# VideoVerses/VideoTuna-dev

Measured on AMD Instinct MI355X. Metric: finetune samples/sec, CogVideoX-2B T2V LoRA 49x480x720 bf16, higher is better.
Workload: dtype bf16; 1 GPU; CogVideoX-2B T2V LoRA finetune 49x480x720 (configs[1]): latents [4,13,16,60,90], text [4,226,4096], r=4 LoRA on to_q/k/v/out, 4 samples per optimizer step as in the YAML (batch_size 2 x accumulate_grad_batches 2), run as 1 micro-batch(es) of 4; mode=lora, model=CogVideoX-2B, micro_batch=4, accumulate_grad_batches=1, global_batch=4, seq_len=17776, layers=30, parallelism=dp1, recompute=none (107 GB of block activations kept in HBM), weights=seeded random init (no checkpoints offline), text=pre-encoded prompt embeddings (synthetic), latents=pre-encoded latents (synthetic)

## Files before the change

include/vt355.h:

```cpp
#ifndef VT355_H
#define VT355_H
#ifdef __cplusplus
extern "C" {
#endif

#define VT_OK 0
#define VT_ERR_BAD_SHAPE (-1)
#define VT_ERR_BAD_ALIGN (-2)
#define VT_ERR_LAUNCH (-3)
#define VT_ERR_UNSUPPORTED (-4)

int vt_version(void);
const char* vt_arch(void);
const char* vt_error_string(int code);

#define VT_EPI_BIAS 0
#define VT_EPI_BIAS_GELU 1
#define VT_EPI_GATED_RES 2
#define VT_EPI_DGELU 3

int vt_gemm_bf16(const void* A, int lda, const void* W, int ldw, void* C, int ldc,
                 int M, int N, int K, const void* bias, int epilogue, int out_fp32,
                 const void* R, int ldr, int r_mod,
                 const float* gate_txt, const float* gate_vid, int gate_bstride, int S, int St,
                 void* C2, int ldc2, const void* U, int ldu, void* stream);
int vt_gemm_set_tile(int mode);
int vt_gemm_bf16_kernel(int M, int N, int K);
int vt_conv_set_tile(int mode);

int vt_gemm_nt_bf16(const void* A, int lda, const void* B, int ldb, float* C, int ldc, int M, int P, int Q,
                    float alpha, int accumulate, void* stream);
int vt_gemm_nt_bf16_unpad(const void* A, int lda, const void* B, int ldb, float* C, int ldc, int M, int P, int Q,
                          float alpha, int accumulate, int row_group, int row_keep, int col_group, int col_keep, void* stream);

int vt_group_colsum(const void* X, int ldx, const void* Y, int ldy, const float* mean, const float* rstd,
                    float* out1, float* out2, long long M, int D, int S, int St, int grouped,
                    long long o_bstride, long long o_segstride, void* stream);

int vt_qk_ln_param_grads(const float* dq_hat, int lddq, const void* dk_hat, int lddk, const void* qkv, int ld,
                         const float* mean, const float* rstd, float* out_2x2x64, long long M, int H,
                         const float* rope_cos, const float* rope_sin, int S, int St, void* stream);
int vt_ln_param_combine(const float* G1, const float* G2, int G, int D, const void* gamma, const void* beta,
                        const float* scale_txt, const float* scale_vid, int bstride, float* dgamma, float* dbeta,
                        float* dshift_txt, float* dshift_vid, float* dscale_txt, float* dscale_vid, int dbstride,
                        int grouped, void* stream);
int vt_small_linear_bwd(const float* dy, int ldy, const void* x, int ldx, const void* W, float* dW, float* db,
                        float* dx, int lddx, int Bn, int N, int K, void* stream);
int vt_silu_bwd(const float* dy, const void* x, float* dx, long long n, void* stream);

int vt_attn_fwd_hd64(const void* q, const void* k, const void* v, void* o, float* lse2,
                     int B, int H, int S,
                     long long q_rs, long long k_rs, long long v_rs, long long o_rs,
                     long long q_bs, long long k_bs, long long v_bs, long long o_bs,
                     float softmax_scale, int q_prescaled, void* stream);

int vt_attn_fwd_bias_hd64(const void* q, const void* k, const void* v, const float* bias_t, void* o, float* lse2,
                          int B, int H, int S,
                          long long q_rs, long long k_rs, long long v_rs, long long o_rs,
                          long long q_bs, long long k_bs, long long v_bs, long long o_bs,
                          float softmax_scale, void* stream);
int vt_gemm_splitk_f32(const void* A, int lda, const void* W, int ldw, float* C, int ldc, int M, int N, int K, int splits, void* stream);
int vt_residual_cast_bf16(const float* acc, long long lda, const void* R, long long ldr, void* out, long long ldo, long long M, int N,
                          void* stream);
long long vt_groupnorm_ws_bytes(int N, int C);
int vt_groupnorm_silu_cl(const void* x, long long ldx, const void* gamma, const void* beta, void* y, long long ldy,
                         int N, long long P, int C, int G, float eps, int silu, float* ws, long long ws_bytes, void* stream);
int vt_causal_conv3d_cl(const void* x, long long ldx, const void* wk, const void* bias, const void* res, long long ldr,
                        void* y, long long ldy, int N, int T, int H, int W, int Cin, int Cout, void* stream);
int vt_downsample_conv2d_cl(const void* x, long long ldx, const void* wk, const void* bias, void* y, long long ldy,
                            int N, int T, int H, int W, int Cin, int Cout, void* stream);
int vt_causal_conv3d_in8_cl(const void* x, const void* wk, const void* bias, void* y, long long ldy,
                            int N, int T, int H, int W, int Cout, void* stream);
int vt_temporal_pool_cl(const void* x, long long ldx, void* y, long long ldy, int N, int T, long long HW, int C, int keep_first,
                        void* stream);
int vt_rmsnorm_bf16(const void* x, long long ldx, const void* w, void* y, long long ldy, long long M, int D, float eps,
                    void* stream);
int vt_gated_gelu_bf16(const void* u, long long ldu, void* y, long long ldy, long long M, int F, void* stream);

int vt_attn_bwd_hd64(const void* q, const void* k, const void* v, const void* o, const void* dout,
                     const float* lse2, float* delta_ws, float* dq_f32, void* dk, void* dv,
                     int B, int H, int S,
                     long long q_rs, long long k_rs, long long v_rs, long long o_rs, long long do_rs,
                     long long dq_rs, long long dk_rs, long long dv_rs,
                     long long q_bs, long long k_bs, long long v_bs, long long o_bs, long long do_bs,
                     long long dq_bs, long long dk_bs, long long dv_bs,
                     float softmax_scale, int q_prescaled, void* chain_ws, long long chain_ws_bytes, void* stream);
long long vt_attn_bwd_chain_ws_bytes(int B, int H, int S);
int vt_attn_bwd_set_chain(int chain_len, int slots);

int vt_ln_modulate_fwd(const void* x, int ldx, void* y, int ldy, const void* gamma, const void* beta,
                       const float* shift_txt, const float* scale_txt, const float* shift_vid,
                       const float* scale_vid, int mod_bstride, float* mean, float* rstd,
                       int M, int D, int S, int St, float eps, void* stream);
int vt_ln_modulate_bwd(const void* dy, int lddy, const void* x, int ldx, const float* mean, const float* rstd,
                       const void* gamma, const float* scale_txt, const float* scale_vid, int mod_bstride,
                       const void* dres, int lddres, void* dx, int lddx,
                       int M, int D, int S, int St, void* stream);

int vt_qk_layernorm_fwd(const void* qkv, int ld, void* out, int ldo, const void* gq, const void* bq,
                        const void* gk, const void* bk, float* mean, float* rstd,
                        long long M, int H, float eps, float q_scale,
                        const float* rope_cos, const float* rope_sin, int S, int St, void* stream);
int vt_qk_layernorm_bwd(const float* dq_hat, int lddq, const void* dk_hat, int lddk, const void* qkv, int ld,
                        const float* mean, const float* rstd, const void* gq, const void* gk,
                        void* dqkv, int ldd, long long M, int H,
                        const float* rope_cos, const float* rope_sin, int S, int St, void* stream);

int vt_gate_mul(const void* x, int ldx, void* y, int ldy, const float* g_txt, const float* g_vid, int bstride,
                long long M, int D, int S, int St, void* stream);
int vt_silu_bf16(const void* x, void* y, long long n, void* stream);
int vt_cast_f32_bf16(const float* x, void* y, long long n, void* stream);
int vt_timestep_embedding(const long long* t, void* out, int B, int D, int flip_sin_to_cos, float freq_shift,
                          void* stream);
int vt_patchify(const void* img, void* tok, int B, int F, int C, int H, int W, int P, int ldt, void* stream);
int vt_unpatchify(const void* tok, void* img, int B, int F, int C, int H, int W, int P, int ldt, void* stream);

int vt_add_noise(const float* x0, const float* noise, const float* sqrt_ab, const float* sqrt_1mab, void* noisy,
                 long long per_sample, int B, void* stream);
int vt_diffusion_loss(const void* vpred, const void* noisy, const float* x0, const float* sqrt_ab,
                      const float* sqrt_1mab, const float* weights, float* loss, float* partials_ws,
                      void* dvpred, long long per_sample, int B, float grad_scale, void* stream);

int vt_diffusion_loss_bwd(const void* vpred, const void* noisy, const float* x0, const float* sqrt_ab,
                          const float* sqrt_1mab, const float* weights, const float* grad_out, void* dvpred,
                          long long per_sample, int B, void* stream);

int vt_adamw(float* p, const float* g, float* m, float* v, void* p_bf16, long long n, float lr, float beta1,
             float beta2, float eps, float weight_decay, int step, float grad_scale, const int* guard, void* stream);

int vt_grad_sqnorm_partials(void);
int vt_grad_sqnorm(const float* g, long long n, float* partials, int slot, void* stream);
int vt_clip_finalize(const float* partials, int nslots, float grad_scale, float max_norm, float* record, void* stream);
int vt_adamw_clip(float* p, const float* g, float* m, float* v, void* p_bf16, long long n, float lr, float beta1,
                  float beta2, float eps, float weight_decay, int step, float grad_scale, const int* guard,
                  const float* clip_coef_dev, float clip_value, void* stream);

int vt_lora_down(const void* X, int ldx, const void* A, int lda, int R, void* T, int ldt, long long M, int K,
                 int zero_cols, void* stream);
int vt_skinny_tn(const void* Big, int ldb, const void* Small, int lds_, int R, float* out, long long osp,
                 long long osr, float alpha, long long M, int P, float* workspace, void* stream);
long long vt_skinny_tn_workspace_bytes(int P);
int vt_lora_up_add(void* dX, int ldx, const void* dT, int ldt, const void* A, int lda, int R, long long M, int K,
                   void* stream);
int vt_lora_pack_b(const float* Bcat, void* Wext, int ldw, int n_adapters, int d_out, int r, float scale, void* stream);
int vt_lora_pack_bt(const float* Bcat, void* WText, int ldwt, int n_adapters, int d_out, int r, float scale, void* stream);

int vt_lora_down_wide(const void* X, int ldx, const void* A, int lda, int n_adapters, int r, int rp, int ext, void* T, int ldt,
                      long long M, int K, void* stream);
int vt_lora_tn_wide(const void* Big, int ldb, const void* Small, int lds_, int R, float* out, long long osp, long long osr,
                    float alpha, long long M, int P, void* stream);
int vt_lora_up_add_wide(void* dX, int ldx, const void* dT, int ldt, const void* A, int lda, int n_adapters, int r, int rp,
                        long long M, int K, void* stream);
int vt_lora_pack_b_wide(const float* Bcat, void* Wext, int ldw, int n_adapters, int d_out, int r, int rp, int ext, float scale,
                        void* stream);
int vt_lora_pack_bt_wide(const float* Bcat, void* WText, int ldwt, int n_adapters, int d_out, int r, int rp, int ext, float scale,
                         void* stream);

int vt_lora_down_drop(const void* X, int ldx, const void* A, int lda, int R, int n_adapters, void* T, int ldt, long long M, int K,
                      int zero_cols, float p, unsigned long long seed, int site0, void* stream);
int vt_skinny_tn_drop(const void* Big, int ldb, const void* Small, int lds_, int R, int n_adapters, float* out, long long osp,
                      long long osr, float alpha, long long M, int P, float* workspace, float p, unsigned long long seed, int site0,
                      void* stream);
int vt_lora_up_add_drop(void* dX, int ldx, const void* dT, int ldt, const void* A, int lda, int R, int n_adapters, long long M, int K,
                        float p, unsigned long long seed, int site0, void* stream);
int vt_lora_down_wide_drop_fits(int n_adapters, int rp);
int vt_lora_down_wide_drop(const void* X, int ldx, const void* A, int lda, int n_adapters, int r, int rp, int ext, void* T, int ldt,
                           long long M, int K, float p, unsigned long long seed, int site0, void* stream);
int vt_lora_tn_wide_drop(const void* Big, int ldb, const void* Small, int lds_, int R, float* out, long long osp, long long osr,
                         float alpha, long long M, int P, float p, unsigned long long seed, int site, void* stream);
int vt_lora_up_add_wide_drop(void* dX, int ldx, const void* dT, int ldt, const void* A, int lda, int n_adapters, int r, int rp,
                             long long M, int K, float p, unsigned long long seed, int site0, void* stream);
int vt_lora_up_add_dgelu_drop(void* dX, int ldx, const void* dT, int ldt, const void* A, int lda, int R, int n_adapters, const void* U,
                              int ldu, long long M, int K, float p, unsigned long long seed, int site0, void* stream);
int vt_lora_up_add_wide_dgelu_drop(void* dX, int ldx, const void* dT, int ldt, const void* A, int lda, int n_adapters, int r, int rp,
                                   const void* U, int ldu, long long M, int K, float p, unsigned long long seed, int site0, void* stream);

int vt_dora_norm(const void* W, int ldw, const void* A, int lda, const void* B, int n_adapters, int d_out, int r, int K, float scale,
                 const float* mag, float* out, void* stream);
int vt_dora_scale(const void* src, long long lds_, void* dst, long long ldd, const float* c, int rows, int cols, int by_col, void* stream);
int vt_dora_transpose_scale(const void* src, long long src_ld, void* dst, long long dst_ld, const float* c, int rows, int cols,
                            void* stream);
int vt_dora_db_add(float* G, const float* S, const float* c, int N, int r, void* stream);
int vt_dora_dm(const float* sum_g, const float* sum_gy, const void* bias, const float* mag, float* dm, int N, void* stream);


int vt_conv_cl(const void* x, long long ldx, const void* wk, const void* bias, const float* sbias, int sbias_ld,
               const void* res, long long ldr, void* y, long long ldy,
               int N, int T, int H, int W, int Cin, int Cout, int KT, int KH, int KW, int pt, int ph, int pw, int stride, void* stream);
int vt_conv_dw_cl(const void* dy, long long lddy, const void* x, long long ldx, float* dw,
                  int N, int T, int H, int W, int Cin, int Cout, int KT, int KH, int KW, int pt, int ph, int pw, int stride,
                  int accumulate, void* stream);
int vt_conv_dw_bias_cl(const void* dy, long long lddy, const void* x, long long ldx, float* dw, float* dbias,
                       int N, int T, int H, int W, int Cin, int Cout, int KT, int KH, int KW, int pt, int ph, int pw, int stride,
                       int accumulate, void* stream);
int vt_transpose_bf16(const void* src, long long src_ld, long long src_boff, void* dst, long long dst_ld, long long dst_boff, int rows, int cols,
                      int nb, void* stream);
int vt_transpose_multi_bf16(const void* table, int njobs, long long total_blocks, void* stream);
int vt_conv_desc_extents(long long ldx, long long lddy, int N, int T, int H, int W, int Cin, int Cout, int KH, int KW, int ph, int pw,
                         int stride, long long* fwd_x_bytes, long long* dw_x_bytes, long long* dw_dy_bytes);
int vt_groupnorm_silu_bwd_cl(const void* dy, long long lddy, const void* x, long long ldx, const void* gamma,
                             const float* ws_fwd, float* ws_bwd, long long ws_bytes, void* dx, long long lddx,
                             float* dgamma, float* dbeta, int N, long long P, int C, int G, int silu, int accumulate, void* stream);
int vt_geglu_fwd(const void* h, long long ldh, void* y, long long ldy, long long M, int F, void* stream);
int vt_geglu_bwd(const void* dy, long long lddy, const void* h, long long ldh, void* dh, long long lddh, long long M, int F, void* stream);
int vt_add_rows_bf16(const void* a, long long lda, const void* b, long long ldb, void* out, long long ldo, long long M, int C, void* stream);
int vt_dropout_bf16(const void* x, long long ldx, void* y, long long ldy, long long M, int C, float p, unsigned long long seed,
                    unsigned long long offset, void* mask_out, void* stream);
int vt_row_map_bf16(const void* src, long long lds, void* out, long long ldo, int mode, long long nb, int d1, int d2, int C,
                    int accumulate, void* stream);
int vt_q_sample(const float* x0, const float* noise, const float* sqrt_ab, const float* sqrt_1mab, const float* scale, void* xt,
                long long per_sample, int B, void* stream);
int vt_mse_loss(const void* pred, const float* target, float* loss, void* dpred, long long total, float grad_scale, void* stream);

int vt_attn_small_fwd(const void* q, const void* k, const void* v, void* o, float* lse2, int NB, int H, int Sq, int Sk,
                      long long q_rs, long long q_bs, long long k_rs, long long k_bs, long long v_rs, long long v_bs,
                      long long o_rs, long long o_bs, float softmax_scale, int mask_block, void* stream);
int vt_attn_small_bwd(const void* q, const void* k, const void* v, const void* o, const void* dout, const float* lse2,
                      void* dq, void* dk, void* dv, float* dk32, float* dv32, int NB, int H, int Sq, int Sk,
                      long long q_rs, long long q_bs, long long k_rs, long long k_bs, long long v_rs, long long v_bs,
                      long long o_rs, long long o_bs, long long do_rs, long long do_bs, long long dq_rs, long long dq_bs,
                      long long dk_rs, long long dv_rs, float softmax_scale, int mask_block, void* stream);

long long vt_attn_dual_ws_floats(int B, int H, int Sq, int rows_per_frame, int Sa, int Sb);
int vt_attn_dual_fwd(const void* q, const void* k, const void* v, const void* k_ip, const void* v_ip, void* o, float* lse2,
                     int B, int H, int Sq, int rows_per_frame, int Sa, int Sb,
                     long long q_rs, long long q_bs, long long k_rs, long long k_bs, long long v_rs, long long v_bs,
                     long long kip_rs, long long kip_bs, long long vip_rs, long long vip_bs, long long o_rs, long long o_bs,
                     float softmax_scale, float img_scale, void* stream);
int vt_attn_dual_bwd(const void* q, const void* k, const void* v, const void* k_ip, const void* v_ip, const void* dout,
                     const float* lse2, void* dq, float* dk32, float* dv32, float* dkip32, float* dvip32, float* ws,
                     long long ws_floats, int B, int H, int Sq, int rows_per_frame, int Sa, int Sb,
                     long long q_rs, long long q_bs, long long k_rs, long long k_bs, long long v_rs, long long v_bs,
                     long long kip_rs, long long kip_bs, long long vip_rs, long long vip_bs, long long do_rs, long long do_bs,
                     long long dq_rs, long long dq_bs, float softmax_scale, float img_scale, void* stream);

int vt_attn_gen_fwd(const void* q, const void* k, const void* v, void* o, float* lse2, const int* kv_len, int head_dim, int hstride,
                    int NB, int H, int Sq, int Sk, long long q_rs, long long q_bs, long long k_rs, long long k_bs, long long v_rs,
                    long long v_bs, long long o_rs, long long o_bs, float softmax_scale, int mask_block, void* stream);
int vt_attn_gen_bwd(const void* q, const void* k, const void* v, const void* o, const void* dout, const float* lse2, const int* kv_len,
                    void* dq, void* dk, void* dv, float* dk32, float* dv32, int head_dim, int hstride, int NB, int H, int Sq, int Sk,
                    long long q_rs, long long q_bs, long long k_rs, long long k_bs, long long v_rs, long long v_bs,
                    long long o_rs, long long o_bs, long long do_rs, long long do_bs, long long dq_rs, long long dq_bs,
                    long long dk_rs, long long dv_rs, float softmax_scale, int mask_block, void* stream);

int vt_opensora_loss(const float* out, const float* x0, const float* noise, const double* coef, double* loss3, float* dout,
                     long long per_channel, int C, int B, float grad_scale, void* stream);

int vt_gemm_fp8(const void* A, int lda, const void* W, int ldw, void* C, int ldc, int M, int N, int K, const void* bias,
                const float* scale_a, const float* scale_w, void* stream);
int vt_quantize_fp8(const void* x, long long ldx, void* y, long long ldy, long long M, int K, float* scale, unsigned int* ws,
                    int given_scale, void* stream);

int vt_gemm_mxfp8(const void* A, int lda, const void* W, int ldw, void* C, int ldc, int M, int N, int K, const void* bias,
                  const float* scale_a, const float* scale_w, int epilogue, const void* residual, int ldr,
                  const float* gate_txt, const float* gate_vid, int gate_bstride, int S, int St, void* pre_act_out, int ldc2,
                  const void* At, int ldat, const void* Wt, int ldwt, int Kt, void* Cq, int ldcq, const float* scale_out,
                  unsigned int* amax, void* stream);
int vt_cast_fp8_scaled(const void* x, long long ldx, void* y, long long ldy, void* cp, long long ldcp, long long M, int K, int L,
                       int Lj, int off, const float* scale, unsigned int* amax, void* stream);
int vt_ln_modulate_fwd_fp8(const void* x, int ldx, void* y, int ldy, const void* gamma, const void* beta,
                           const float* shift_txt, const float* scale_txt, const float* shift_vid,
                           const float* scale_vid, int mod_bstride, float* mean, float* rstd,
                           int M, int D, int S, int St, float eps, void* q, int ldq, const float* qscale, unsigned int* amax,
                           void* stream);
int vt_fp8_scale_update(unsigned int* amax, float* history, float* scale, int n, int H, void* stream);
int vt_gemm_mxfp8_dx(const void* G, int ldg, int fmt_g, const void* WT, int ldw, void* C, int ldc, int M, int N, int K,
                     const float* scale_g, const float* scale_w, int epilogue, const void* residual, int ldr,
                     const void* pre_act_in, int ldu, const void* At, int ldat, const void* Wt, int ldwt, int Kt,
                     void* Cq, int ldcq, int fmt_out, const float* scale_out, unsigned int* amax, void* stream);
int vt_cast_fp8_fmt(const void* x, long long ldx, void* y, long long ldy, void* cp, long long ldcp, long long M, int K, int L,
                    int Lj, int off, int fmt, const float* scale, unsigned int* amax, void* stream);
int vt_gate_mul_fp8(const void* x, int ldx, void* y, int ldy, const float* g_txt, const float* g_vid, int bstride, long long M,
                    int D, int S, int St, void* q, int ldq, int fmt, const float* scale, unsigned int* amax, void* stream);
int vt_fp8_scale_update_fmax(unsigned int* amax, float* history, float* scale, int n, int H, float fmax, void* stream);

int vt_qk_rmsnorm_rope128_fwd(const void* qkv, long long ld, void* out, long long ldo, const void* gq, const void* gk, float* rstd,
                              const float* rope_cos, const float* rope_sin, long long M, int H, int L, int Lout, int row_off,
                              int S_rope, float eps, void* stream);
int vt_qk_rmsnorm_rope128_bwd(const void* dout, long long lddo, const void* qkv, long long ld, void* dqkv, long long ldd, const void* gq,
                              const void* gk, const float* rstd, const float* rope_cos, const float* rope_sin, float* dgq, float* dgk,
                              long long M, int H, int L, int Lout, int row_off, int S_rope, void* stream);

int vt_attn128_fwd(const void* q, const void* k, const void* v, void* o, float* lse2, const int* kv_len, int B, int H, int S,
                   long long q_rs, long long k_rs, long long v_rs, long long o_rs,
                   long long q_bs, long long k_bs, long long v_bs, long long o_bs, float softmax_scale, void* stream);
int vt_attn128_bwd(const void* q, const void* k, const void* v, const void* o, const void* dout, const float* lse2, const int* kv_len,
                   float* delta_ws, float* dq32, void* dq_bf16, void* dk, void* dv, int B, int H, int S,
                   long long q_rs, long long k_rs, long long v_rs, long long o_rs, long long do_rs, long long dq_rs, long long dqb_rs,
                   long long dk_rs, long long dv_rs, long long q_bs, long long k_bs, long long v_bs, long long o_bs, long long do_bs,
                   long long dq_bs, long long dqb_bs, long long dk_bs, long long dv_bs, float softmax_scale, void* stream);

#ifdef __cplusplus
}
#endif
#endif
```

videotuna-dev_amd/_lib.py:

```python
import ctypes as C
import os

_HERE = os.path.dirname(os.path.abspath(__file__))
_LIB = None


class VtError(RuntimeError):
    pass


def lib_path() -> str:
    return os.environ.get("VT355_LIB") or os.path.join(_HERE, "libvt355.so")


_vp, _i, _ll, _f, _fp = C.c_void_p, C.c_int, C.c_longlong, C.c_float, C.c_void_p
PROTOTYPES = {
    "vt_version": [],
    "vt_arch": [],
    "vt_error_string": [_i],
    "vt_gemm_bf16": [_vp, _i, _vp, _i, _vp, _i, _i, _i, _i, _vp, _i, _i, _vp, _i, _i, _fp, _fp, _i, _i, _i,
                     _vp, _i, _vp, _i, _vp],
    "vt_gemm_set_tile": [_i],
    "vt_gemm_bf16_kernel": [_i, _i, _i],
    "vt_conv_set_tile": [_i],
    "vt_transpose_bf16": [_vp, _ll, _ll, _vp, _ll, _ll, _i, _i, _i, _vp],
    "vt_transpose_multi_bf16": [_vp, _i, _ll, _vp],
    "vt_gemm_nt_bf16": [_vp, _i, _vp, _i, _fp, _i, _i, _i, _i, _f, _i, _vp],
    "vt_gemm_nt_bf16_unpad": [_vp, _i, _vp, _i, _fp, _i, _i, _i, _i, _f, _i, _i, _i, _i, _i, _vp],
    "vt_group_colsum": [_vp, _i, _vp, _i, _fp, _fp, _fp, _fp, _ll, _i, _i, _i, _i, _ll, _ll, _vp],
    "vt_qk_ln_param_grads": [_fp, _i, _vp, _i, _vp, _i, _fp, _fp, _fp, _ll, _i, _fp, _fp, _i, _i, _vp],
    "vt_ln_param_combine": [_fp, _fp, _i, _i, _vp, _vp, _fp, _fp, _i, _fp, _fp, _fp, _fp, _fp, _fp, _i, _i, _vp],
    "vt_small_linear_bwd": [_fp, _i, _vp, _i, _vp, _fp, _fp, _fp, _i, _i, _i, _i, _vp],
    "vt_silu_bwd": [_fp, _vp, _fp, _ll, _vp],
    "vt_attn_fwd_hd64": [_vp, _vp, _vp, _vp, _fp, _i, _i, _i, _ll, _ll, _ll, _ll, _ll, _ll, _ll, _ll, _f, _i, _vp],
    "vt_attn_fwd_bias_hd64": [_vp, _vp, _vp, _fp, _vp, _fp, _i, _i, _i, _ll, _ll, _ll, _ll, _ll, _ll, _ll, _ll, _f, _vp],
    "vt_gemm_splitk_f32": [_vp, _i, _vp, _i, _fp, _i, _i, _i, _i, _i, _vp],
    "vt_residual_cast_bf16": [_fp, _ll, _vp, _ll, _vp, _ll, _ll, _i, _vp],
    "vt_groupnorm_ws_bytes": [_i, _i],
    "vt_groupnorm_silu_cl": [_vp, _ll, _vp, _vp, _vp, _ll, _i, _ll, _i, _i, _f, _i, _fp, _ll, _vp],
    "vt_causal_conv3d_cl": [_vp, _ll, _vp, _vp, _vp, _ll, _vp, _ll, _i, _i, _i, _i, _i, _i, _vp],
    "vt_causal_conv3d_in8_cl": [_vp, _vp, _vp, _vp, _ll, _i, _i, _i, _i, _i, _vp],
    "vt_downsample_conv2d_cl": [_vp, _ll, _vp, _vp, _vp, _ll, _i, _i, _i, _i, _i, _i, _vp],
    "vt_temporal_pool_cl": [_vp, _ll, _vp, _ll, _i, _i, _ll, _i, _i, _vp],
    "vt_rmsnorm_bf16": [_vp, _ll, _vp, _vp, _ll, _ll, _i, _f, _vp],
    "vt_gated_gelu_bf16": [_vp, _ll, _vp, _ll, _ll, _i, _vp],
    "vt_attn_bwd_hd64": [_vp, _vp, _vp, _vp, _vp, _fp, _fp, _fp, _vp, _vp, _i, _i, _i,
                         _ll, _ll, _ll, _ll, _ll, _ll, _ll, _ll, _ll, _ll, _ll, _ll, _ll, _ll, _ll, _ll, _f, _i, _vp, _ll, _vp],
    "vt_attn_bwd_chain_ws_bytes": [_i, _i, _i],
    "vt_attn_bwd_set_chain": [_i, _i],
    "vt_ln_modulate_fwd": [_vp, _i, _vp, _i, _vp, _vp, _fp, _fp, _fp, _fp, _i, _fp, _fp, _i, _i, _i, _i, _f, _vp],
    "vt_ln_modulate_bwd": [_vp, _i, _vp, _i, _fp, _fp, _vp, _fp, _fp, _i, _vp, _i, _vp, _i, _i, _i, _i, _i, _vp],
    "vt_qk_layernorm_fwd": [_vp, _i, _vp, _i, _vp, _vp, _vp, _vp, _fp, _fp, _ll, _i, _f, _f, _fp, _fp, _i, _i, _vp],
    "vt_qk_layernorm_bwd": [_fp, _i, _vp, _i, _vp, _i, _fp, _fp, _vp, _vp, _vp, _i, _ll, _i, _fp, _fp, _i, _i, _vp],
    "vt_gate_mul": [_vp, _i, _vp, _i, _fp, _fp, _i, _ll, _i, _i, _i, _vp],
    "vt_silu_bf16": [_vp, _vp, _ll, _vp],
    "vt_cast_f32_bf16": [_fp, _vp, _ll, _vp],
    "vt_timestep_embedding": [_vp, _vp, _i, _i, _i, _f, _vp],
    "vt_patchify": [_vp, _vp, _i, _i, _i, _i, _i, _i, _i, _vp],
    "vt_unpatchify": [_vp, _vp, _i, _i, _i, _i, _i, _i, _i, _vp],
    "vt_add_noise": [_fp, _fp, _fp, _fp, _vp, _ll, _i, _vp],
    "vt_diffusion_loss": [_vp, _vp, _fp, _fp, _fp, _fp, _fp, _fp, _vp, _ll, _i, _f, _vp],
    "vt_diffusion_loss_bwd": [_vp, _vp, _fp, _fp, _fp, _fp, _fp, _vp, _ll, _i, _vp],
    "vt_adamw": [_fp, _fp, _fp, _fp, _vp, _ll, _f, _f, _f, _f, _f, _i, _f, _vp, _vp],
    "vt_grad_sqnorm_partials": [],
    "vt_grad_sqnorm": [_fp, _ll, _fp, _i, _vp],
    "vt_clip_finalize": [_fp, _i, _f, _f, _fp, _vp],
    "vt_adamw_clip": [_fp, _fp, _fp, _fp, _vp, _ll, _f, _f, _f, _f, _f, _i, _f, _vp, _fp, _f, _vp],
    "vt_lora_down": [_vp, _i, _vp, _i, _i, _vp, _i, _ll, _i, _i, _vp],
    "vt_skinny_tn": [_vp, _i, _vp, _i, _i, _fp, _ll, _ll, _f, _ll, _i, _fp, _vp],
    "vt_skinny_tn_workspace_bytes": [_i],
    "vt_lora_up_add": [_vp, _i, _vp, _i, _vp, _i, _i, _ll, _i, _vp],
    "vt_lora_pack_b": [_fp, _vp, _i, _i, _i, _i, _f, _vp],
    "vt_lora_pack_bt": [_fp, _vp, _i, _i, _i, _i, _f, _vp],
    "vt_lora_down_wide": [_vp, _i, _vp, _i, _i, _i, _i, _i, _vp, _i, _ll, _i, _vp],
    "vt_lora_tn_wide": [_vp, _i, _vp, _i, _i, _fp, _ll, _ll, _f, _ll, _i, _vp],
    "vt_lora_up_add_wide": [_vp, _i, _vp, _i, _vp, _i, _i, _i, _i, _ll, _i, _vp],
    "vt_lora_pack_b_wide": [_fp, _vp, _i, _i, _i, _i, _i, _i, _f, _vp],
    "vt_lora_pack_bt_wide": [_fp, _vp, _i, _i, _i, _i, _i, _i, _f, _vp],
    "vt_lora_down_drop": [_vp, _i, _vp, _i, _i, _i, _vp, _i, _ll, _i, _i, _f, C.c_ulonglong, _i, _vp],
    "vt_skinny_tn_drop": [_vp, _i, _vp, _i, _i, _i, _fp, _ll, _ll, _f, _ll, _i, _fp, _f, C.c_ulonglong, _i, _vp],
    "vt_lora_up_add_drop": [_vp, _i, _vp, _i, _vp, _i, _i, _i, _ll, _i, _f, C.c_ulonglong, _i, _vp],
    "vt_lora_down_wide_drop_fits": [_i, _i],
    "vt_lora_down_wide_drop": [_vp, _i, _vp, _i, _i, _i, _i, _i, _vp, _i, _ll, _i, _f, C.c_ulonglong, _i, _vp],
    "vt_lora_tn_wide_drop": [_vp, _i, _vp, _i, _i, _fp, _ll, _ll, _f, _ll, _i, _f, C.c_ulonglong, _i, _vp],
    "vt_lora_up_add_wide_drop": [_vp, _i, _vp, _i, _vp, _i, _i, _i, _i, _ll, _i, _f, C.c_ulonglong, _i, _vp],
    "vt_lora_up_add_dgelu_drop": [_vp, _i, _vp, _i, _vp, _i, _i, _i, _vp, _i, _ll, _i, _f, C.c_ulonglong, _i, _vp],
    "vt_lora_up_add_wide_dgelu_drop": [_vp, _i, _vp, _i, _vp, _i, _i, _i, _i, _vp, _i, _ll, _i, _f, C.c_ulonglong, _i, _vp],
    "vt_dora_norm": [_vp, _i, _vp, _i, _vp, _i, _i, _i, _i, _f, _fp, _fp, _vp],
    "vt_dora_scale": [_vp, _ll, _vp, _ll, _fp, _i, _i, _i, _vp],
    "vt_dora_transpose_scale": [_vp, _ll, _vp, _ll, _fp, _i, _i, _vp],
    "vt_dora_db_add": [_fp, _fp, _fp, _i, _i, _vp],
    "vt_dora_dm": [_fp, _fp, _vp, _fp, _fp, _i, _vp],
    "vt_conv_cl": [_vp, _ll, _vp, _vp, _fp, _i, _vp, _ll, _vp, _ll] + [_i] * 13 + [_vp],
    "vt_conv_dw_cl": [_vp, _ll, _vp, _ll, _fp] + [_i] * 13 + [_i, _vp],
    "vt_conv_dw_bias_cl": [_vp, _ll, _vp, _ll, _fp, _fp] + [_i] * 13 + [_i, _vp],
    "vt_conv_desc_extents": [_ll, _ll] + [_i] * 11 + [C.POINTER(C.c_longlong)] * 3,
    "vt_groupnorm_silu_bwd_cl": [_vp, _ll, _vp, _ll, _vp, _fp, _fp, _ll, _vp, _ll, _fp, _fp, _i, _ll, _i, _i, _i, _i, _vp],
    "vt_geglu_fwd": [_vp, _ll, _vp, _ll, _ll, _i, _vp],
    "vt_geglu_bwd": [_vp, _ll, _vp, _ll, _vp, _ll, _ll, _i, _vp],
    "vt_add_rows_bf16": [_vp, _ll, _vp, _ll, _vp, _ll, _ll, _i, _vp],
    "vt_dropout_bf16": [_vp, _ll, _vp, _ll, _ll, _i, _f, C.c_ulonglong, C.c_ulonglong, _vp, _vp],
    "vt_row_map_bf16": [_vp, _ll, _vp, _ll, _i, _ll, _i, _i, _i, _i, _vp],
    "vt_q_sample": [_fp, _fp, _fp, _fp, _fp, _vp, _ll, _i, _vp],
    "vt_mse_loss": [_vp, _fp, _fp, _vp, _ll, _f, _vp],
    "vt_attn_small_fwd": [_vp, _vp, _vp, _vp, _fp, _i, _i, _i, _i] + [_ll] * 8 + [_f, _i, _vp],
    "vt_qk_rmsnorm_rope128_fwd": [_vp, _ll, _vp, _ll, _vp, _vp, _fp, _fp, _fp, _ll, _i, _i, _i, _i, _i, _f, _vp],
    "vt_qk_rmsnorm_rope128_bwd": [_vp, _ll, _vp, _ll, _vp, _ll, _vp, _vp, _fp, _fp, _fp, _fp, _fp, _ll, _i, _i, _i, _i, _i, _vp],
    "vt_attn128_fwd": [_vp, _vp, _vp, _vp, _fp, _vp, _i, _i, _i] + [_ll] * 8 + [_f, _vp],
    "vt_attn128_bwd": [_vp, _vp, _vp, _vp, _vp, _fp, _vp, _fp, _fp, _vp, _vp, _vp, _i, _i, _i] + [_ll] * 18 + [_f, _vp],
    "vt_gemm_fp8": [_vp, _i, _vp, _i, _vp, _i, _i, _i, _i, _vp, _fp, _fp, _vp],
    "vt_quantize_fp8": [_vp, _ll, _vp, _ll, _ll, _i, _fp, _vp, _i, _vp],
    "vt_gemm_mxfp8": [_vp, _i, _vp, _i, _vp, _i, _i, _i, _i, _vp, _fp, _fp, _i, _vp, _i, _fp, _fp, _i, _i, _i, _vp, _i,
                      _vp, _i, _vp, _i, _i, _vp, _i, _fp, _vp, _vp],
    "vt_cast_fp8_scaled": [_vp, _ll, _vp, _ll, _vp, _ll, _ll, _i, _i, _i, _i, _fp, _vp, _vp],
    "vt_ln_modulate_fwd_fp8": [_vp, _i, _vp, _i, _vp, _vp, _fp, _fp, _fp, _fp, _i, _fp, _fp, _i, _i, _i, _i, _f, _vp, _i, _fp, _vp, _vp],
    "vt_fp8_scale_update": [_vp, _fp, _fp, _i, _i, _vp],
    "vt_gemm_mxfp8_dx": [_vp, _i, _i, _vp, _i, _vp, _i, _i, _i, _i, _fp, _fp, _i, _vp, _i, _vp, _i, _vp, _i, _vp, _i, _i,
                         _vp, _i, _i, _fp, _vp, _vp],
    "vt_cast_fp8_fmt": [_vp, _ll, _vp, _ll, _vp, _ll, _ll, _i, _i, _i, _i, _i, _fp, _vp, _vp],
    "vt_gate_mul_fp8": [_vp, _i, _vp, _i, _fp, _fp, _i, _ll, _i, _i, _i, _vp, _i, _i, _fp, _vp, _vp],
    "vt_fp8_scale_update_fmax": [_vp, _fp, _fp, _i, _i, _f, _vp],
    "vt_opensora_loss": [_fp, _fp, _fp, _vp, _vp, _fp, _ll, _i, _i, _f, _vp],
    "vt_attn_gen_fwd": [_vp, _vp, _vp, _vp, _fp, _vp, _i, _i, _i, _i, _i, _i] + [_ll] * 8 + [_f, _i, _vp],
    "vt_attn_gen_bwd": [_vp, _vp, _vp, _vp, _vp, _fp, _vp, _vp, _vp, _vp, _fp, _fp, _i, _i, _i, _i, _i, _i] + [_ll] * 14 + [_f, _i, _vp],
    "vt_attn_small_bwd": [_vp, _vp, _vp, _vp, _vp, _fp, _vp, _vp, _vp, _fp, _fp, _i, _i, _i, _i] + [_ll] * 14 + [_f, _i, _vp],
    "vt_attn_dual_ws_floats": [_i] * 6,
    "vt_attn_dual_fwd": [_vp] * 6 + [_fp] + [_i] * 6 + [_ll] * 12 + [_f, _f, _vp],
    "vt_attn_dual_bwd": [_vp] * 6 + [_fp, _vp] + [_fp] * 5 + [_ll] + [_i] * 6 + [_ll] * 14 + [_f, _f, _vp],
}
_RESTYPE = {"vt_arch": C.c_char_p, "vt_error_string": C.c_char_p, "vt_skinny_tn_workspace_bytes": C.c_longlong,
             "vt_attn_bwd_chain_ws_bytes": C.c_longlong, "vt_groupnorm_ws_bytes": C.c_longlong,
             "vt_attn_dual_ws_floats": C.c_longlong}


def load_library():
    global _LIB
    if _LIB is not None:
        return _LIB
    import torch
    path = lib_path()
    if not os.path.exists(path):
        raise VtError(f"{path} not found: build it with `python -c 'import __graft_entry__ as g; g.build()'` "
                      f"(videotuna-dev_amd/csrc/build.sh). There is no CPU / eager fallback.")
    lib = C.CDLL(path)
    for name, args in PROTOTYPES.items():
        fn = getattr(lib, name)
        fn.argtypes = args
        fn.restype = _RESTYPE.get(name, C.c_int)
    _LIB = lib
    return lib


def check(code: int, what: str):
    if code != 0:
        lib = load_library()
        raise VtError(f"{what} failed: {lib.vt_error_string(code).decode()} (code {code})")
```

videotuna-dev_amd/csrc/attn_bwd.hip:

```cpp
#include "common.h"
#include <cstdlib>

#ifndef VT_SUFFIX
#define VT_SUFFIX
#endif
#ifndef VT_CLK
#define VT_CLK 0
#endif
#define VT_CAT_(a, b) a##b
#define VT_CAT(a, b) VT_CAT_(a, b)
#define BWD_KERNEL VT_CAT(attn_bwd_hd64_kernel, VT_SUFFIX)
#define BWD_BODY VT_CAT(attn_bwd_body, VT_SUFFIX)
#define DELTA_KERNEL VT_CAT(attn_bwd_delta_kernel, VT_SUFFIX)
#define BWD_ENTRY VT_CAT(vt_attn_bwd_hd64, VT_SUFFIX)

#define BWD_THREADS 512
#define FENCE() __builtin_amdgcn_sched_barrier(0)
#define DQ_RING 2
#define PF_TRN 4
#define PF_ROWN 2

struct AttnBwdParams {
    const bf16_t* q;
    const bf16_t* k;
// ... 412 lines not shown
            bf16_t* dvp = p.dv + (size_t)b * p.dv_bs + (size_t)key * p.dv_rs + head * 64;
#pragma unroll
            for (int dt = 0; dt < 4; ++dt) {
                u32x2 a, c;
                a[0] = pack2(dk16[dt][kt][0] * dk_mul, dk16[dt][kt][1] * dk_mul);
                a[1] = pack2(dk16[dt][kt][2] * dk_mul, dk16[dt][kt][3] * dk_mul);
                c[0] = pack2(dv16[dt][kt][0], dv16[dt][kt][1]);
                c[1] = pack2(dv16[dt][kt][2], dv16[dt][kt][3]);
                *(u32x2*)(dkp + 16 * dt + 4 * g) = a;
                *(u32x2*)(dvp + 16 * dt + 4 * g) = c;
            }
        }
    }
}


#if VT_CLK
__device__ unsigned VT_CAT(vt_bwd_clk, VT_SUFFIX)[4];
extern "C" int VT_CAT(vt_attn_bwd_clk, VT_SUFFIX)(unsigned* host_out) {
    return hipMemcpyFromSymbol(host_out, HIP_SYMBOL(VT_CAT(vt_bwd_clk, VT_SUFFIX)), 4 * sizeof(unsigned)) == hipSuccess ? VT_OK : VT_ERR_LAUNCH;
}
#endif
template <bool PRESCALED>
__global__ __launch_bounds__(BWD_THREADS, 1) void BWD_KERNEL(AttnBwdParams p) {
    __shared__ __attribute__((aligned(16))) char smem[BWD_LDS];
    __shared__ __attribute__((aligned(16))) char stage[CH_STAGE_BYTES];
    const int nkb = (p.S + 255) / 256;
    const int nitems = nkb * p.H * p.B, nsteps = (p.S + 63) / 64;
    const int L = p.chain_len;
    const int spx = gridDim.x >> 3;
    const int slot = (int)(blockIdx.x & 7) * spx + (int)(blockIdx.x >> 3);
    bool dead = false;
    int cons_end = 0;
    int gen = 0;
    bool l2_prev = false, l2_next = false;
    if (L > 1) {
        int xcc;
        asm volatile("s_getreg_b32 %0, hwreg(HW_REG_XCC_ID)" : "=s"(xcc));
        xcc = (xcc & 15) + 1;
        __amdgpu_buffer_rsrc_t rx = make_rsrc(p.chain_xcc, (unsigned)gridDim.x * 4u);
        if (threadIdx.x == 0) __builtin_amdgcn_raw_buffer_store_b32((unsigned)xcc, rx, slot * 4, 0, CH_AUX);
        const int j = slot % spx;
        auto peer = [&](int s2) -> int {
            int v = 0, it = 0;
            while (v == 0 && it++ < (1 << 16)) {
                v = __builtin_amdgcn_readfirstlane((int)__builtin_amdgcn_raw_buffer_load_b32(rx, s2 * 4, 0, CH_AUX));
                if (v == 0) __builtin_amdgcn_s_sleep(8);
            }
            return v;
        };
        if ((j % L) != 0) {
            l2_prev = peer(slot - 1) == xcc;
            if (threadIdx.x == 0) atomicAdd(p.chain_ctr + (l2_prev ? 11 : 12), 1);
        }
        if ((j % L) != L - 1 && j != spx - 1 && slot + 1 < (int)gridDim.x) l2_next = peer(slot + 1) == xcc;
    }
    for (int item = slot; item < nitems; item += gridDim.x, ++gen) {
        const int kblk = item % nkb;
        bool has_prod = false, has_cons = false;
        if (L > 1) {
            const int j = slot % spx;
            has_prod = (j % L) != 0 && kblk != 0;
            has_cons = (j % L) != L - 1 && j != spx - 1 && kblk != nkb - 1 && item + 1 < nitems;
        }
        const bool ragged = (kblk + 1) * 256 > p.S;
        const int role = (has_prod ? 1 : 0) | (has_cons ? 2 : 0);
        const int base = gen * nsteps;
#define VT_BWD_CALL(R, ROLE_) BWD_BODY<R, PRESCALED, ROLE_>(p, smem, stage, item, slot, cons_end, base, l2_prev, l2_next, dead)
#if VT_CLK
        unsigned long long clk0, rt0;
        asm volatile("s_memtime %0\n\ts_memrealtime %1\n\ts_waitcnt lgkmcnt(0)" : "=s"(clk0), "=s"(rt0) :: "memory");
#endif
        switch (role) {
            case 0: if (ragged) VT_BWD_CALL(true, 0); else VT_BWD_CALL(false, 0); break;
            case 1: if (ragged) VT_BWD_CALL(true, 1); else VT_BWD_CALL(false, 1); break;
            case 2: VT_BWD_CALL(false, 2); break;
            default: VT_BWD_CALL(false, 3); break;
        }
#undef VT_BWD_CALL
#if VT_CLK
        {
            unsigned long long clk1, rt1;
            asm volatile("s_memtime %0\n\ts_memrealtime %1\n\ts_waitcnt lgkmcnt(0)" : "=s"(clk1), "=s"(rt1) :: "memory");
            if (blockIdx.x == 40 && gen == 3 && threadIdx.x == 0) {
                VT_CAT(vt_bwd_clk, VT_SUFFIX)[0] = (unsigned)(clk1 - clk0);
                VT_CAT(vt_bwd_clk, VT_SUFFIX)[1] = (unsigned)(rt1 - rt0);
            }
        }
#endif
        if (has_cons) cons_end = (gen + 1) * nsteps;
        __syncthreads();
    }
}

__global__ __launch_bounds__(256) void DELTA_KERNEL(const bf16_t* o, const bf16_t* dout, float* delta,
                                                            int B, int H, int S, long long o_rs, long long do_rs,
                                                            long long o_bs, long long do_bs) {
    const long long gid = (long long)blockIdx.x * 256 + threadIdx.x;
    const long long row = gid >> 3;
    const int sub = (int)(gid & 7);
    const long long total = (long long)B * S * H;
    float acc = 0.f;
    long long bs = 0; int hh = 0;
    if (row < total) {
        hh = (int)(row % H);
        bs = row / H;
        const int s = (int)(bs % S);
        const int b = (int)(bs / S);
        u32x4 a = *(const u32x4*)(o + (size_t)b * o_bs + (size_t)s * o_rs + hh * 64 + sub * 8);
        u32x4 c = *(const u32x4*)(dout + (size_t)b * do_bs + (size_t)s * do_rs + hh * 64 + sub * 8);
        float fa[8], fc[8];
        unpack8(a, fa);
        unpack8(c, fc);
#pragma unroll
        for (int i = 0; i < 8; ++i) acc += fa[i] * fc[i];
    }
    acc += __shfl_xor(acc, 1, 64);
    acc += __shfl_xor(acc, 2, 64);
    acc += __shfl_xor(acc, 4, 64);
    if (row < total && sub == 0) {
        const int s = (int)(bs % S);
        const int b = (int)(bs / S);
        delta[((size_t)b * H + hh) * S + s] = acc;
    }
}

static long long bwd_chain_xcc_off(long long slots) { return 256 + slots * 64; }
static long long bwd_chain_tiles_off(long long slots) { return (256 + slots * 68 + 4095) & ~4095LL; }
static long long bwd_chain_ws_bytes(long long slots) { return bwd_chain_tiles_off(slots) + slots * (long long)(CH_R * 16384); }
static int g_bwd_slots = 0;
static int g_bwd_chain = -1;
static void bwd_chain_init() {
    if (g_bwd_chain >= 0) return;
    int L = 3;
    if (const char* e = getenv("VT_BWD_CHAIN")) L = atoi(e);
    int dev = 0, cus = 0;
    if (hipGetDevice(&dev) != hipSuccess || hipDeviceGetAttribute(&cus, hipDeviceAttributeMultiprocessorCount, dev) != hipSuccess) cus = 0;
    g_bwd_slots = cus / 8 * 8;
    if (g_bwd_slots < 8) g_bwd_slots = 8;
    g_bwd_chain = L < 1 ? 1 : L;
}
static int bwd_chain_len() { bwd_chain_init(); return g_bwd_chain; }
extern "C" int VT_CAT(vt_attn_bwd_set_chain, VT_SUFFIX)(int chain_len, int slots) {
    g_bwd_chain = -1;
    bwd_chain_init();
    if (chain_len > 0) g_bwd_chain = chain_len;
    if (slots > 0) {
        if ((slots % 8) || slots > g_bwd_slots) return VT_ERR_BAD_SHAPE;
        g_bwd_slots = slots;
    }
    return VT_OK;
}

extern "C" int BWD_ENTRY(const void* q, const void* k, const void* v, const void* o, const void* dout,
                                const float* lse2, float* delta_ws, float* dq_f32, void* dk, void* dv,
                                int B, int H, int S,
                                long long q_rs, long long k_rs, long long v_rs, long long o_rs, long long do_rs,
                                long long dq_rs, long long dk_rs, long long dv_rs,
                                long long q_bs, long long k_bs, long long v_bs, long long o_bs, long long do_bs,
                                long long dq_bs, long long dk_bs, long long dv_bs,
                                float softmax_scale, int q_prescaled, void* chain_ws, long long chain_ws_bytes,
                                void* stream) {
    if (B <= 0 || H <= 0 || S <= 0) return VT_ERR_BAD_SHAPE;
    if ((long long)S * dq_rs * 4 >= 0x7fffffffLL) return VT_ERR_BAD_SHAPE;
    if ((q_rs % 8) || (k_rs % 8) || (v_rs % 8) || (o_rs % 8) || (do_rs % 8) || (dk_rs % 4) || (dv_rs % 4)) return VT_ERR_BAD_SHAPE;
    if ((q_bs % 8) || (k_bs % 8) || (v_bs % 8) || (o_bs % 8) || (do_bs % 8) || (dk_bs % 4) || (dv_bs % 4)) return VT_ERR_BAD_SHAPE;
    if ((((uintptr_t)q) | ((uintptr_t)k) | ((uintptr_t)v) | ((uintptr_t)o) | ((uintptr_t)dout)) & 15) return VT_ERR_BAD_ALIGN;
    if ((((uintptr_t)dk) | ((uintptr_t)dv)) & 7) return VT_ERR_BAD_ALIGN;
    const long long lim = 0x7fffffffLL;
    if ((long long)S * q_rs * 2 >= lim || (long long)S * k_rs * 2 >= lim || (long long)S * v_rs * 2 >= lim ||
        (long long)S * do_rs * 2 >= lim) return VT_ERR_BAD_SHAPE;
    hipStream_t st = (hipStream_t)stream;
    {
        const long long total = (long long)B * S * H * 8;
        const int blocks = (int)((total + 255) / 256);
        hipLaunchKernelGGL(DELTA_KERNEL, dim3(blocks), dim3(256), 0, st, (const bf16_t*)o, (const bf16_t*)dout,
                           delta_ws, B, H, S, o_rs, do_rs, o_bs, do_bs);
    }
    AttnBwdParams p;
    p.q = (const bf16_t*)q; p.k = (const bf16_t*)k; p.v = (const bf16_t*)v; p.dout = (const bf16_t*)dout;
    p.lse2 = lse2; p.delta = delta_ws; p.dq = dq_f32; p.dk = (bf16_t*)dk; p.dv = (bf16_t*)dv;
    p.S = S; p.H = H; p.B = B;
    p.q_rs = q_rs; p.k_rs = k_rs; p.v_rs = v_rs; p.do_rs = do_rs; p.dq_rs = dq_rs; p.dk_rs = dk_rs; p.dv_rs = dv_rs;
    p.q_bs = q_bs; p.k_bs = k_bs; p.v_bs = v_bs; p.do_bs = do_bs; p.dq_bs = dq_bs; p.dk_bs = dk_bs; p.dv_bs = dv_bs;
    p.scale = softmax_scale; p.scale_log2 = softmax_scale * 1.4426950408889634f;
    const int nkb = (S + 255) / 256;
    const long long nwg = (long long)nkb * H * B;
    if (nwg > 0x3fffffLL) return VT_ERR_BAD_SHAPE;
    p.chain_len = 1; p.chain_ctr = nullptr; p.chain_flags = nullptr; p.chain_xcc = nullptr; p.chain_tiles = nullptr;
    int L = bwd_chain_len();
    const long long pgrid = nwg < g_bwd_slots ? (nwg + 7) / 8 * 8 : g_bwd_slots;
    const long long grid = pgrid;
    if (L > pgrid / 8) L = (int)(pgrid / 8);
    if (L > nkb) L = nkb;
    if (chain_ws != nullptr && chain_ws_bytes >= 64 && !(((uintptr_t)chain_ws) & 255)) {
        char* ws = (char*)chain_ws;
        const bool on = L > 1 && chain_ws_bytes >= bwd_chain_ws_bytes(g_bwd_slots);
        if (hipMemsetAsync(ws, 0, 64, st) != hipSuccess) return VT_ERR_LAUNCH;
        if (on && hipMemsetAsync(ws + 256, 0, (size_t)bwd_chain_tiles_off(g_bwd_slots) - 256, st) != hipSuccess) return VT_ERR_LAUNCH;
        if (on) {
            p.chain_len = L;
            p.chain_ctr = (int*)ws;
            p.chain_flags = (int*)(ws + 256);
            p.chain_xcc = (int*)(ws + bwd_chain_xcc_off(g_bwd_slots));
            p.chain_tiles = (float*)(ws + bwd_chain_tiles_off(g_bwd_slots));
        }
    }
    if (q_prescaled) hipLaunchKernelGGL(BWD_KERNEL<true>, dim3((unsigned)grid), dim3(BWD_THREADS), 0, st, p);
    else hipLaunchKernelGGL(BWD_KERNEL<false>, dim3((unsigned)grid), dim3(BWD_THREADS), 0, st, p);
    return hipGetLastError() == hipSuccess ? VT_OK : VT_ERR_LAUNCH;
}

extern "C" long long VT_CAT(vt_attn_bwd_chain_ws_bytes, VT_SUFFIX)(int B, int H, int S) {
    if (B <= 0 || H <= 0 || S <= 0 || bwd_chain_len() <= 1) return 0;
    return bwd_chain_ws_bytes(g_bwd_slots);
}
```

videotuna-dev_amd/csrc/lora.hip:

```cpp
#include "common.h"
#include <cstdlib>

static int lora_drop_args_bad(int R, int n, float p, int site0) {
    return n <= 0 || n > 3 || R <= 0 || R > 16 || (R % n) || vt_lora_drop_bad(p, site0);
}

template <typename... D>
__global__ __launch_bounds__(256) void lora_down_kernel(const bf16_t* X, int ldx, const bf16_t* A, int lda, int R,
                                                       bf16_t* T, int ldt, long long M, int K, int zero_cols, D... drop) {
    constexpr bool DROP = sizeof...(D) > 0;
    const LoraDrop dr = lora_drop_arg(drop...);
    const int lane = threadIdx.x & 63, wave = threadIdx.x >> 6;
    const long long row0 = ((long long)blockIdx.x * 4 + wave) * 16;
    if (row0 >= M) return;
    const int fr = lane & 15, fq = lane >> 4;
    long long xr = row0 + fr;
    if (xr > M - 1) xr = M - 1;
    const bf16_t* xp = X + (size_t)xr * ldx + 16 * fq;
    const bool aok = fr < R;
    const bf16_t* ap = A + (size_t)(aok ? fr : 0) * lda + 16 * fq;
    const int ja = DROP ? fr / dr.r : 0;
    const unsigned long long e4 = DROP ? ((unsigned long long)xr * K + 16 * fq) >> 2 : 0;
    f32x4 acc = {0.f, 0.f, 0.f, 0.f};
    const u32x4 zero = {0u, 0u, 0u, 0u};
// ... 128 lines not shown
        const int pb0 = blockIdx.x * 512;
#pragma unroll
        for (int c = 0; c < 4; ++c)
#pragma unroll
            for (int rr = 0; rr < RR; ++rr) sm[(pl + c) * RR + rr] = alpha * acc[c][rr];
        __syncthreads();
        if (osr == 1) {
            for (int i = threadIdx.x; i < 512 * RR; i += 128) {
                const int pp = i / RR, rr = i - pp * RR;
                if (rr < R && pb0 + pp < P) atomicAdd(out + (size_t)(pb0 + pp) * osp + rr, sm[i]);
            }
        } else {
            for (int rr = 0; rr < R; ++rr)
                for (int pp = threadIdx.x; pp < 512; pp += 128)
                    if (pb0 + pp < P) atomicAdd(out + (size_t)(pb0 + pp) * osp + (size_t)rr * osr, sm[pp * RR + rr]);
        }
    }
}
template <int RR>
__global__ __launch_bounds__(256) void skinny_reduce_kernel(const float* ws, int nslices, float* out, long long osp, long long osr,
                                                           float alpha, int P, int R) {
    const int i = blockIdx.x * 256 + threadIdx.x;
    if (i >= P * RR) return;
    const int p = i / RR, rr = i - p * RR;
    if (rr >= R) return;
    float s = 0.f;
    for (int k = 0; k < nslices; ++k) s += ws[(size_t)k * P * RR + i];
    out[(size_t)p * osp + (size_t)rr * osr] += alpha * s;
}
extern "C" long long vt_skinny_tn_workspace_bytes(int P) { return (long long)SK_COPIES * P * 16 * 4; }
#define SK_ARGS bg, ldb, smp, lds_, R, out, osp, osr, alpha, mc, P, rps, workspace
#define SK_DROP_LAUNCH(RR_, NA_, RPER_) \
    hipLaunchKernelGGL((skinny_tn_kernel<RR_, NA_, RPER_, LoraDrop>), grid, dim3(128), 0, st, SK_ARGS, drm)
static int skinny_tn_launch(const void* Big, int ldb, const void* Small, int lds_, int R, float* out, long long osp, long long osr,
                            float alpha, long long M, int P, float* workspace, int nsl, const LoraDrop* dr, void* stream) {
    if (M <= 0 || P <= 0 || (P % 4) || R <= 0 || R > 16 || (ldb % 4)) return VT_ERR_BAD_SHAPE;
    if (((uintptr_t)Big) & 7) return VT_ERR_BAD_ALIGN;
    if (workspace != nullptr && (((uintptr_t)workspace) & 15)) return VT_ERR_BAD_ALIGN;
    hipStream_t st = (hipStream_t)stream;
    const long long chunk = (long long)nsl * SK_MAXROWS;
    const int RRw = R <= 4 ? 4 : 16;
    if (workspace != nullptr && hipMemsetAsync(workspace, 0, (size_t)SK_COPIES * P * RRw * 4, st) != hipSuccess) return VT_ERR_LAUNCH;
    for (long long mbase = 0; mbase < M; mbase += chunk) {
        const long long mc = (M - mbase) < chunk ? (M - mbase) : chunk;
        const int rps = (int)((mc + nsl - 1) / nsl);
        dim3 grid((P + 511) / 512, nsl);
        const bf16_t* bg = (const bf16_t*)Big + (size_t)mbase * ldb;
        const bf16_t* smp = (const bf16_t*)Small + (size_t)mbase * lds_;
        if (dr == nullptr) {
            if (R <= 4) hipLaunchKernelGGL((skinny_tn_kernel<4, 0, 1>), grid, dim3(128), 0, st, SK_ARGS);
            else hipLaunchKernelGGL((skinny_tn_kernel<16, 0, 1>), grid, dim3(128), 0, st, SK_ARGS);
        } else {
            LoraDrop drm = *dr;
            drm.mbase = mbase;
            if (dr->n == 1) {
                if (R <= 4) SK_DROP_LAUNCH(4, 1, 16); else SK_DROP_LAUNCH(16, 1, 16);
            } else if (dr->r == 1) SK_DROP_LAUNCH(4, 3, 1);
            else if (dr->r == 2) SK_DROP_LAUNCH(16, 3, 2);
            else if (dr->r == 3) SK_DROP_LAUNCH(16, 3, 3);
            else if (dr->r == 4) SK_DROP_LAUNCH(16, 3, 4);
            else SK_DROP_LAUNCH(16, 3, 5);
        }
    }
    if (workspace != nullptr) {
        if (R <= 4) hipLaunchKernelGGL(skinny_reduce_kernel<4>, dim3((P * 4 + 255) / 256), dim3(256), 0, st, workspace, SK_COPIES, out, osp, osr, alpha, P, R);
        else hipLaunchKernelGGL(skinny_reduce_kernel<16>, dim3((P * 16 + 255) / 256), dim3(256), 0, st, workspace, SK_COPIES, out, osp, osr, alpha, P, R);
    }
    return hipGetLastError() == hipSuccess ? VT_OK : VT_ERR_LAUNCH;
}
#undef SK_DROP_LAUNCH
#undef SK_ARGS
extern "C" int vt_skinny_tn(const void* Big, int ldb, const void* Small, int lds_, int R, float* out, long long osp,
                            long long osr, float alpha, long long M, int P, float* workspace, void* stream) {
    static int slices_env = -1;
    if (slices_env < 0) { const char* e = getenv("VT_SK_SLICES"); slices_env = e ? atoi(e) : 0; }
    const int nsl = (slices_env > 0 && slices_env <= 1024) ? slices_env : SK_SLICES;
    return skinny_tn_launch(Big, ldb, Small, lds_, R, out, osp, osr, alpha, M, P, workspace, nsl, nullptr, stream);
}
extern "C" int vt_skinny_tn_drop(const void* Big, int ldb, const void* Small, int lds_, int R, int n_adapters, float* out, long long osp,
                                 long long osr, float alpha, long long M, int P, float* workspace, float p, unsigned long long seed,
                                 int site0, void* stream) {
    if (lora_drop_args_bad(R, n_adapters, p, site0) || n_adapters == 2) return VT_ERR_BAD_SHAPE;
    const LoraDrop dr = vt_lora_drop(p, seed, site0, n_adapters, R / n_adapters);
    return skinny_tn_launch(Big, ldb, Small, lds_, R, out, osp, osr, alpha * dr.inv_keep, M, P, workspace, SK_SLICES, &dr, stream);
}

template <typename... D>
__global__ __launch_bounds__(256) void lora_up_add_kernel(bf16_t* dX, int ldx, const bf16_t* dT, int ldt, const bf16_t* A, int lda,
                                                         int R, long long M, int K, D... drop) {
    constexpr bool DROP = sizeof...(D) > 0, DGELU = sizeof...(D) > 1;
    const LoraDrop dr = lora_drop_arg(drop...);
    const LoraDgelu dg = lora_dgelu_arg(drop...);
    const int n = DROP ? dr.n : 1, r = DROP ? dr.r : R;
    const int nch = K >> 3;
    const long long total = M * nch;
    for (long long i = (long long)blockIdx.x * 256 + threadIdx.x; i < total; i += (long long)gridDim.x * 256) {
        const long long m = i / nch;
        const int c = (int)(i - m * nch);
        float v[8];
        unpack8(*(const u32x4*)(dX + (size_t)m * ldx + c * 8), v);
        float g[8];
        if constexpr (DGELU) {
            unpack8(*(const u32x4*)(dg.U + (size_t)m * dg.ldu + c * 8), g);
#pragma unroll
            for (int q = 0; q < 8; ++q) g[q] = dr.inv_keep * gelu_tanh_grad_f(g[q]);
        }
        for (int j = 0; j < n; ++j) {
            float s[8] = {0.f, 0.f, 0.f, 0.f, 0.f, 0.f, 0.f, 0.f};
            float(&acc)[8] = DROP ? s : v;
            for (int ri = j * r; ri < (j + 1) * r; ++ri) {
                const float t = bf2f(dT[(size_t)m * ldt + ri]);
                float a[8];
                unpack8(*(const u32x4*)(A + (size_t)ri * lda + c * 8), a);
#pragma unroll
                for (int q = 0; q < 8; ++q) acc[q] += t * a[q];
            }
            if constexpr (DROP) {
                unsigned rnd[8];
                const unsigned long long ctr = lora_site_offset(dr.site0 + j) + (((unsigned long long)m * K + 8 * c) >> 2);
                keep_words4(ctr, dr.seed, rnd);
                keep_words4(ctr + 1, dr.seed, rnd + 4);
#pragma unroll
                for (int q = 0; q < 8; ++q) v[q] += rnd[q] >= dr.thresh ? (DGELU ? g[q] : dr.inv_keep) * s[q] : 0.f;
            }
        }
        *(u32x4*)(dX + (size_t)m * ldx + c * 8) = pack8(v);
    }
}
static int lora_up_add_launch(void* dX, int ldx, const void* dT, int ldt, const void* A, int lda, int R, long long M, int K,
                              const LoraDrop* dr, void* stream, const LoraDgelu* dg = nullptr) {
    if (M <= 0 || K <= 0 || (K % 8) || R <= 0 || R > 16 || (ldx % 8) || (lda % 8)) return VT_ERR_BAD_SHAPE;
    if ((((uintptr_t)dX) | ((uintptr_t)A)) & 15) return VT_ERR_BAD_ALIGN;
    if (dg != nullptr) {
        if (dr == nullptr || dg->U == nullptr || (dg->ldu % 8) || dg->ldu < K || ldx < K || ldt < R) return VT_ERR_BAD_SHAPE;
        if (((uintptr_t)dg->U) & 15) return VT_ERR_BAD_ALIGN;
    }
    long long total = M * (K >> 3), b = (total + 255) / 256;
    const dim3 grid((unsigned)(b > 8192 ? 8192 : b));
    if (dr == nullptr)
        hipLaunchKernelGGL(lora_up_add_kernel<>, grid, dim3(256), 0, (hipStream_t)stream, (bf16_t*)dX, ldx, (const bf16_t*)dT, ldt,
                           (const bf16_t*)A, lda, R, M, K);
    else if (dg != nullptr)
        hipLaunchKernelGGL((lora_up_add_kernel<LoraDrop, LoraDgelu>), grid, dim3(256), 0, (hipStream_t)stream, (bf16_t*)dX, ldx,
                           (const bf16_t*)dT, ldt, (const bf16_t*)A, lda, R, M, K, *dr, *dg);
    else
        hipLaunchKernelGGL(lora_up_add_kernel<LoraDrop>, grid, dim3(256), 0, (hipStream_t)stream, (bf16_t*)dX, ldx, (const bf16_t*)dT, ldt,
                           (const bf16_t*)A, lda, R, M, K, *dr);
    return hipGetLastError() == hipSuccess ? VT_OK : VT_ERR_LAUNCH;
}
extern "C" int vt_lora_up_add(void* dX, int ldx, const void* dT, int ldt, const void* A, int lda, int R, long long M, int K,
                              void* stream) {
    return lora_up_add_launch(dX, ldx, dT, ldt, A, lda, R, M, K, nullptr, stream);
}
extern "C" int vt_lora_up_add_drop(void* dX, int ldx, const void* dT, int ldt, const void* A, int lda, int R, int n_adapters, long long M,
                                   int K, float p, unsigned long long seed, int site0, void* stream) {
    if (lora_drop_args_bad(R, n_adapters, p, site0)) return VT_ERR_BAD_SHAPE;
    const LoraDrop dr = vt_lora_drop(p, seed, site0, n_adapters, R / n_adapters);
    return lora_up_add_launch(dX, ldx, dT, ldt, A, lda, R, M, K, &dr, stream);
}
extern "C" int vt_lora_up_add_dgelu_drop(void* dX, int ldx, const void* dT, int ldt, const void* A, int lda, int R, int n_adapters,
                                         const void* U, int ldu, long long M, int K, float p, unsigned long long seed, int site0,
                                         void* stream) {
    if (lora_drop_args_bad(R, n_adapters, p, site0)) return VT_ERR_BAD_SHAPE;
    const LoraDrop dr = vt_lora_drop(p, seed, site0, n_adapters, R / n_adapters);
    const LoraDgelu dg = {(const bf16_t*)U, ldu};
    return lora_up_add_launch(dX, ldx, dT, ldt, A, lda, R, M, K, &dr, stream, &dg);
}

__global__ void lora_pack_b_kernel(const float* Bcat, bf16_t* Wext, int ldw, int n_adapters, int d_out, int r, float scale) {
    const int i = blockIdx.x * 256 + threadIdx.x;
    const int total = n_adapters * d_out * 64;
    if (i >= total) return;
    const int n = i >> 6, c = i & 63;
    const int j = n / d_out;
    float v = 0.f;
    if (c >= j * r && c < (j + 1) * r) v = scale * Bcat[(size_t)n * r + (c - j * r)];
    Wext[(size_t)n * ldw + c] = f2bf(v);
}
extern "C" int vt_lora_pack_b(const float* Bcat, void* Wext, int ldw, int n_adapters, int d_out, int r, float scale,
                              void* stream) {
    if (n_adapters <= 0 || d_out <= 0 || r <= 0 || n_adapters * r > 64) return VT_ERR_BAD_SHAPE;
    const int total = n_adapters * d_out * 64;
    hipLaunchKernelGGL(lora_pack_b_kernel, dim3((total + 255) / 256), dim3(256), 0, (hipStream_t)stream, Bcat, (bf16_t*)Wext, ldw,
                       n_adapters, d_out, r, scale);
    return hipGetLastError() == hipSuccess ? VT_OK : VT_ERR_LAUNCH;
}

__global__ void lora_pack_bt_kernel(const float* Bcat, bf16_t* WText, int ldwt, int n_adapters, int d_out, int r, float scale) {
    const int i = blockIdx.x * 256 + threadIdx.x;
    const int N = n_adapters * d_out;
    if (i >= 64 * N) return;
    const int c = i / N, n = i - c * N;
    const int j = n / d_out;
    float v = 0.f;
    if (c >= j * r && c < (j + 1) * r) v = scale * Bcat[(size_t)n * r + (c - j * r)];
    WText[(size_t)c * ldwt + n] = f2bf(v);
}
extern "C" int vt_lora_pack_bt(const float* Bcat, void* WText, int ldwt, int n_adapters, int d_out, int r, float scale,
                               void* stream) {
    if (n_adapters <= 0 || d_out <= 0 || r <= 0 || n_adapters * r > 64) return VT_ERR_BAD_SHAPE;
    const int total = n_adapters * d_out * 64;
    hipLaunchKernelGGL(lora_pack_bt_kernel, dim3((total + 255) / 256), dim3(256), 0, (hipStream_t)stream, Bcat, (bf16_t*)WText, ldwt,
                       n_adapters, d_out, r, scale);
    return hipGetLastError() == hipSuccess ? VT_OK : VT_ERR_LAUNCH;
}
```

videotuna-dev_amd/csrc/norm.hip:

```cpp
#include "common.h"

#define LN_MAXCH 8

struct LnParams {
    const bf16_t* x; int ldx;
    bf16_t* y; int ldy;
    const bf16_t* gamma; const bf16_t* beta;
    const float* shift_txt; const float* scale_txt; const float* shift_vid; const float* scale_vid;
    int mod_bstride;
    float* mean; float* rstd;
    int M, D, S, St;
    float eps;
    unsigned char* q; int ldq; const float* qscale; unsigned int* amax;
};

template <int NCH, bool Q = false>
__global__ __launch_bounds__(256) void ln_modulate_fwd_kernel(LnParams p) {
    const int lane = threadIdx.x & 63;
    const int m = blockIdx.x * 4 + (threadIdx.x >> 6);
    if (m >= p.M) return;
    const int nchunks = p.D >> 3;
    const bf16_t* xr = p.x + (size_t)m * p.ldx;
    float v[NCH][8];
    float sum = 0.f;
#pragma unroll
    for (int i = 0; i < NCH; ++i) {
        const int c = lane + 64 * i;
        if (c < nchunks) {
            u32x4 raw = *(const u32x4*)(xr + c * 8);
            unpack8(raw, v[i]);
#pragma unroll
            for (int j = 0; j < 8; ++j) sum += v[i][j];
        } else {
#pragma unroll
            for (int j = 0; j < 8; ++j) v[i][j] = 0.f;
        }
    }
    const float mean = wave_sum(sum) / (float)p.D;
    float sq = 0.f;
#pragma unroll
    for (int i = 0; i < NCH; ++i) {
        const int c = lane + 64 * i;
        if (c < nchunks) {
#pragma unroll
            for (int j = 0; j < 8; ++j) { float d = v[i][j] - mean; sq += d * d; }
        }
    }
    const float rstd = rsqrtf(wave_sum(sq) / (float)p.D + p.eps);
    if (lane == 0 && p.mean != nullptr) { p.mean[m] = mean; p.rstd[m] = rstd; }
    const float* sh = nullptr; const float* scp = nullptr;
    if (p.shift_vid != nullptr) {
        const int b = m / p.S;
        const int s = m - b * p.S;
        sh = (s < p.St ? p.shift_txt : p.shift_vid) + (size_t)b * p.mod_bstride;
        scp = (s < p.St ? p.scale_txt : p.scale_vid) + (size_t)b * p.mod_bstride;
    }
    bf16_t* yr = p.y + (size_t)m * p.ldy;
    float qmax = 0.f;
#pragma unroll
    for (int i = 0; i < NCH; ++i) {
        const int c = lane + 64 * i;
        if (c < nchunks) {
            float o[8];
            float ga[8], be[8];
            if (p.gamma != nullptr) {
                unpack8(*(const u32x4*)(p.gamma + c * 8), ga);
                unpack8(*(const u32x4*)(p.beta + c * 8), be);
            }
#pragma unroll
            for (int j = 0; j < 8; ++j) {
                float t = (v[i][j] - mean) * rstd;
                if (p.gamma != nullptr) t = t * ga[j] + be[j];
                o[j] = t;
            }
            if (sh != nullptr) {
                f32x4 s0 = *(const f32x4*)(scp + c * 8), s1 = *(const f32x4*)(scp + c * 8 + 4);
                f32x4 h0 = *(const f32x4*)(sh + c * 8), h1 = *(const f32x4*)(sh + c * 8 + 4);
#pragma unroll
                for (int j = 0; j < 4; ++j) {
                    o[j] = o[j] * (1.f + s0[j]) + h0[j];
                    o[j + 4] = o[j + 4] * (1.f + s1[j]) + h1[j];
                }
            }
            const u32x4 packed = pack8(o);
            *(u32x4*)(yr + c * 8) = packed;
            if constexpr (Q) {
                float b[8];
                unpack8(packed, b);
                const float qs = p.qscale[0];
                unsigned int w[2];
#pragma unroll
                for (int h = 0; h < 2; ++h) {
                    float t[4];
#pragma unroll
                    for (int j = 0; j < 4; ++j) {
                        qmax = fmaxf(qmax, fabsf(b[4 * h + j]));
                        t[j] = fminf(fmaxf(__fdiv_rn(b[4 * h + j], qs), -448.0f), 448.0f);
                    }
                    int r = 0;
                    r = __builtin_amdgcn_cvt_pk_fp8_f32(t[0], t[1], r, false);
                    r = __builtin_amdgcn_cvt_pk_fp8_f32(t[2], t[3], r, true);
                    w[h] = (unsigned int)r;
                }
                *(u32x2*)(p.q + (size_t)m * p.ldq + c * 8) = (u32x2){w[0], w[1]};
            }
        }
    }
    if constexpr (Q) {
        qmax = wave_max(qmax);
        if (lane == 0) amax_publish(p.amax, qmax);
    }
}

struct LnBwdParams {
    const bf16_t* dy; int lddy;
    const bf16_t* x; int ldx;
    const float* mean; const float* rstd;
    const bf16_t* gamma;
    const float* scale_txt; const float* scale_vid; int mod_bstride;
    const bf16_t* dres; int lddres;
    bf16_t* dx; int lddx;
    int M, D, S, St;
};

template <int NCH>
__global__ __launch_bounds__(256) void ln_modulate_bwd_kernel(LnBwdParams p) {
    const int lane = threadIdx.x & 63;
    const int m = blockIdx.x * 4 + (threadIdx.x >> 6);
    if (m >= p.M) return;
    const int nchunks = p.D >> 3;
    const float mean = p.mean[m], rstd = p.rstd[m];
    const float* scp = nullptr;
    if (p.scale_vid != nullptr) {
        const int b = m / p.S;
        const int s = m - b * p.S;
        scp = (s < p.St ? p.scale_txt : p.scale_vid) + (size_t)b * p.mod_bstride;
    }
    float gv[NCH][8], xh[NCH][8];
    float s1 = 0.f, s2 = 0.f;
#pragma unroll
    for (int i = 0; i < NCH; ++i) {
        const int c = lane + 64 * i;
        if (c < nchunks) {
            float dyv[8], xv[8];
            unpack8(*(const u32x4*)(p.dy + (size_t)m * p.lddy + c * 8), dyv);
            unpack8(*(const u32x4*)(p.x + (size_t)m * p.ldx + c * 8), xv);
            float ga[8];
            if (p.gamma != nullptr) unpack8(*(const u32x4*)(p.gamma + c * 8), ga);
            float sc8[8];
            if (scp != nullptr) {
                f32x4 a = *(const f32x4*)(scp + c * 8), bq = *(const f32x4*)(scp + c * 8 + 4);
#pragma unroll
                for (int j = 0; j < 4; ++j) { sc8[j] = 1.f + a[j]; sc8[j + 4] = 1.f + bq[j]; }
            }
#pragma unroll
            for (int j = 0; j < 8; ++j) {
                float gg = dyv[j];
                if (scp != nullptr) gg *= sc8[j];
                if (p.gamma != nullptr) gg *= ga[j];
                float xhat = (xv[j] - mean) * rstd;
                gv[i][j] = gg;
                xh[i][j] = xhat;
                s1 += gg;
                s2 += gg * xhat;
            }
        } else {
#pragma unroll
            for (int j = 0; j < 8; ++j) { gv[i][j] = 0.f; xh[i][j] = 0.f; }
        }
    }
    const float invD = 1.f / (float)p.D;
    const float m1 = wave_sum(s1) * invD, m2 = wave_sum(s2) * invD;
#pragma unroll
    for (int i = 0; i < NCH; ++i) {
        const int c = lane + 64 * i;
        if (c < nchunks) {
            float o[8];
#pragma unroll
            for (int j = 0; j < 8; ++j) o[j] = rstd * (gv[i][j] - m1 - xh[i][j] * m2);
            if (p.dres != nullptr) {
                float dr[8];
                unpack8(*(const u32x4*)(p.dres + (size_t)m * p.lddres + c * 8), dr);
#pragma unroll
                for (int j = 0; j < 8; ++j) o[j] += dr[j];
            }
            *(u32x4*)(p.dx + (size_t)m * p.lddx + c * 8) = pack8(o);
        }
    }
}

static int nch_for(int D) { return ((D >> 3) + 63) / 64; }

extern "C" int vt_ln_modulate_fwd(const void* x, int ldx, void* y, int ldy, const void* gamma, const void* beta,
                                  const float* shift_txt, const float* scale_txt, const float* shift_vid,
                                  const float* scale_vid, int mod_bstride, float* mean, float* rstd,
                                  int M, int D, int S, int St, float eps, void* stream) {
    if (M <= 0 || D <= 0 || (D % 8) || D > 4096 || (ldx % 8) || (ldy % 8)) return VT_ERR_BAD_SHAPE;
    if ((gamma == nullptr) != (beta == nullptr)) return VT_ERR_BAD_SHAPE;
    if (shift_vid != nullptr && (shift_txt == nullptr || scale_txt == nullptr || scale_vid == nullptr || (mod_bstride % 4)))
        return VT_ERR_BAD_SHAPE;
    if ((((uintptr_t)x) | ((uintptr_t)y)) & 15) return VT_ERR_BAD_ALIGN;
    LnParams p{(const bf16_t*)x, ldx, (bf16_t*)y, ldy, (const bf16_t*)gamma, (const bf16_t*)beta,
               shift_txt, scale_txt, shift_vid, scale_vid, mod_bstride, mean, rstd, M, D, S > 0 ? S : 1, St, eps};
    dim3 grid((M + 3) / 4), block(256);
    hipStream_t st = (hipStream_t)stream;
    const int nch = nch_for(D);
    if (nch <= 1) hipLaunchKernelGGL(ln_modulate_fwd_kernel<1>, grid, block, 0, st, p);
    else if (nch <= 4) hipLaunchKernelGGL(ln_modulate_fwd_kernel<4>, grid, block, 0, st, p);
    else hipLaunchKernelGGL(ln_modulate_fwd_kernel<8>, grid, block, 0, st, p);
    return hipGetLastError() == hipSuccess ? VT_OK : VT_ERR_LAUNCH;
}

extern "C" int vt_ln_modulate_fwd_fp8(const void* x, int ldx, void* y, int ldy, const void* gamma, const void* beta,
                                      const float* shift_txt, const float* scale_txt, const float* shift_vid,
                                      const float* scale_vid, int mod_bstride, float* mean, float* rstd,
                                      int M, int D, int S, int St, float eps, void* q, int ldq, const float* qscale, unsigned int* amax,
                                      void* stream) {
    if (M <= 0 || D <= 0 || (D % 8) || D > 4096 || (ldx % 8) || (ldy % 8) || (ldq % 8) || ldq < D) return VT_ERR_BAD_SHAPE;
    if (q == nullptr || qscale == nullptr || amax == nullptr) return VT_ERR_BAD_SHAPE;
    if ((gamma == nullptr) != (beta == nullptr)) return VT_ERR_BAD_SHAPE;
    if (shift_vid != nullptr && (shift_txt == nullptr || scale_txt == nullptr || scale_vid == nullptr || (mod_bstride % 4)))
        return VT_ERR_BAD_SHAPE;
    if ((((uintptr_t)x) | ((uintptr_t)y)) & 15 || (((uintptr_t)q) & 7)) return VT_ERR_BAD_ALIGN;
    LnParams p{(const bf16_t*)x, ldx, (bf16_t*)y, ldy, (const bf16_t*)gamma, (const bf16_t*)beta,
               shift_txt, scale_txt, shift_vid, scale_vid, mod_bstride, mean, rstd, M, D, S > 0 ? S : 1, St, eps,
               (unsigned char*)q, ldq, qscale, amax};
    dim3 grid((M + 3) / 4), block(256);
    hipStream_t st = (hipStream_t)stream;
    const int nch = nch_for(D);
    if (nch <= 1) hipLaunchKernelGGL((ln_modulate_fwd_kernel<1, true>), grid, block, 0, st, p);
    else if (nch <= 4) hipLaunchKernelGGL((ln_modulate_fwd_kernel<4, true>), grid, block, 0, st, p);
    else hipLaunchKernelGGL((ln_modulate_fwd_kernel<8, true>), grid, block, 0, st, p);
    return hipGetLastError() == hipSuccess ? VT_OK : VT_ERR_LAUNCH;
}

extern "C" int vt_ln_modulate_bwd(const void* dy, int lddy, const void* x, int ldx, const float* mean, const float* rstd,
                                  const void* gamma, const float* scale_txt, const float* scale_vid, int mod_bstride,
                                  const void* dres, int lddres, void* dx, int lddx,
                                  int M, int D, int S, int St, void* stream) {
    if (M <= 0 || D <= 0 || (D % 8) || D > 4096 || (ldx % 8) || (lddy % 8) || (lddx % 8)) return VT_ERR_BAD_SHAPE;
    if (dres != nullptr && (lddres % 8)) return VT_ERR_BAD_SHAPE;
    if (scale_vid != nullptr && (scale_txt == nullptr || (mod_bstride % 4))) return VT_ERR_BAD_SHAPE;
    if ((((uintptr_t)x) | ((uintptr_t)dy) | ((uintptr_t)dx) | ((uintptr_t)dres)) & 15) return VT_ERR_BAD_ALIGN;
    LnBwdParams p{(const bf16_t*)dy, lddy, (const bf16_t*)x, ldx, mean, rstd, (const bf16_t*)gamma,
                  scale_txt, scale_vid, mod_bstride, (const bf16_t*)dres, lddres, (bf16_t*)dx, lddx,
                  M, D, S > 0 ? S : 1, St};
    dim3 grid((M + 3) / 4), block(256);
    hipStream_t st = (hipStream_t)stream;
    const int nch = nch_for(D);
    if (nch <= 1) hipLaunchKernelGGL(ln_modulate_bwd_kernel<1>, grid, block, 0, st, p);
    else if (nch <= 4) hipLaunchKernelGGL(ln_modulate_bwd_kernel<4>, grid, block, 0, st, p);
    else hipLaunchKernelGGL(ln_modulate_bwd_kernel<8>, grid, block, 0, st, p);
    return hipGetLastError() == hipSuccess ? VT_OK : VT_ERR_LAUNCH;
}

__global__ __launch_bounds__(256) void qk_layernorm_fwd_kernel(const bf16_t* qkv, int ld, bf16_t* out, int ldo,
                                                              const bf16_t* gq, const bf16_t* bq, const bf16_t* gk,
                                                              const bf16_t* bk, float* mean, float* rstd,
                                                              long long M, int H, float eps, float q_scale,
                                                              const float* rope_cos, const float* rope_sin, int S, int St) {
    const long long gid = (long long)blockIdx.x * 256 + threadIdx.x;
    const long long grp = gid >> 3;
    const int sub = (int)(gid & 7);
    const long long total = M * 2 * H;
    const bool ok = grp < total;
    const long long m = ok ? grp / (2 * H) : 0;
    const int wh = ok ? (int)(grp % (2 * H)) : 0;
    float v[8];
    if (ok) unpack8(*(const u32x4*)(qkv + (size_t)m * ld + wh * 64 + sub * 8), v);
    else {
#pragma unroll
        for (int j = 0; j < 8; ++j) v[j] = 0.f;
    }
    float s = 0.f;
#pragma unroll
    for (int j = 0; j < 8; ++j) s += v[j];
    s += __shfl_xor(s, 1, 64); s += __shfl_xor(s, 2, 64); s += __shfl_xor(s, 4, 64);
    const float mu = s * (1.f / 64.f);
    float q = 0.f;
#pragma unroll
    for (int j = 0; j < 8; ++j) { float d = v[j] - mu; q += d * d; }
    q += __shfl_xor(q, 1, 64); q += __shfl_xor(q, 2, 64); q += __shfl_xor(q, 4, 64);
    const float rs = rsqrtf(q * (1.f / 64.f) + eps);
    if (!ok) return;
    const bool isk = wh >= H;
    float ga[8], be[8];
    unpack8(*(const u32x4*)((isk ? gk : gq) + sub * 8), ga);
    unpack8(*(const u32x4*)((isk ? bk : bq) + sub * 8), be);
    const float osc = isk ? 1.0f : q_scale;
    float o[8];
#pragma unroll
    for (int j = 0; j < 8; ++j) o[j] = (v[j] - mu) * rs * ga[j] + be[j];
    const int spos = rope_cos != nullptr ? (int)(m % S) - St : -1;
    if (spos >= 0) {
        float cs[8], sn[8];
        rope_load8(rope_cos + (size_t)spos * 64 + sub * 8, cs);
        rope_load8(rope_sin + (size_t)spos * 64 + sub * 8, sn);
#pragma unroll
        for (int j = 0; j < 8; j += 2) {
            const float a = o[j], b = o[j + 1];
            o[j] = a * cs[j] - b * sn[j];
            o[j + 1] = b * cs[j + 1] + a * sn[j + 1];
        }
    }
#pragma unroll
    for (int j = 0; j < 8; ++j) o[j] *= osc;
    *(u32x4*)(out + (size_t)m * ldo + wh * 64 + sub * 8) = pack8(o);
    if (sub == 0) { mean[m * 2 * H + wh] = mu; rstd[m * 2 * H + wh] = rs; }
}

__global__ __launch_bounds__(256) void qk_layernorm_bwd_kernel(const float* dqh, int lddq, const bf16_t* dkh, int lddk,
                                                              const bf16_t* qkv, int ld, const float* mean,
                                                              const float* rstd, const bf16_t* gq, const bf16_t* gk,
                                                              bf16_t* dqkv, int ldd, long long M, int H,
                                                              const float* rope_cos, const float* rope_sin, int S, int St) {
    const long long gid = (long long)blockIdx.x * 256 + threadIdx.x;
    const long long grp = gid >> 3;
    const int sub = (int)(gid & 7);
    const long long total = M * 2 * H;
    const bool ok = grp < total;
    const long long m = ok ? grp / (2 * H) : 0;
    const int wh = ok ? (int)(grp % (2 * H)) : 0;
    const bool isk = wh >= H;
    float g[8], xh[8];
    float mu = 0.f, rs = 0.f;
    if (ok) {
        mu = mean[m * 2 * H + wh];
        rs = rstd[m * 2 * H + wh];
        float dy[8], xv[8], ga[8];
        if (isk) {
            unpack8(*(const u32x4*)(dkh + (size_t)m * lddk + (wh - H) * 64 + sub * 8), dy);
        } else {
            const float* src = dqh + (size_t)m * lddq + wh * 64 + sub * 8;
            f32x4 a = *(const f32x4*)src, b = *(const f32x4*)(src + 4);
#pragma unroll
            for (int j = 0; j < 4; ++j) { dy[j] = a[j]; dy[j + 4] = b[j]; }
        }
        const int spos = rope_cos != nullptr ? (int)(m % S) - St : -1;
        if (spos >= 0) rope_bwd8(rope_cos, rope_sin, spos, sub, dy);
        unpack8(*(const u32x4*)(qkv + (size_t)m * ld + wh * 64 + sub * 8), xv);
        unpack8(*(const u32x4*)((isk ? gk : gq) + sub * 8), ga);
#pragma unroll
        for (int j = 0; j < 8; ++j) { g[j] = dy[j] * ga[j]; xh[j] = (xv[j] - mu) * rs; }
    } else {
#pragma unroll
        for (int j = 0; j < 8; ++j) { g[j] = 0.f; xh[j] = 0.f; }
    }
    float s1 = 0.f, s2 = 0.f;
#pragma unroll
    for (int j = 0; j < 8; ++j) { s1 += g[j]; s2 += g[j] * xh[j]; }
    s1 += __shfl_xor(s1, 1, 64); s1 += __shfl_xor(s1, 2, 64); s1 += __shfl_xor(s1, 4, 64);
    s2 += __shfl_xor(s2, 1, 64); s2 += __shfl_xor(s2, 2, 64); s2 += __shfl_xor(s2, 4, 64);
    if (!ok) return;
    const float m1 = s1 * (1.f / 64.f), m2 = s2 * (1.f / 64.f);
    float o[8];
#pragma unroll
    for (int j = 0; j < 8; ++j) o[j] = rs * (g[j] - m1 - xh[j] * m2);
    *(u32x4*)(dqkv + (size_t)m * ldd + wh * 64 + sub * 8) = pack8(o);
}

extern "C" int vt_qk_layernorm_fwd(const void* qkv, int ld, void* out, int ldo, const void* gq, const void* bq,
                                   const void* gk, const void* bk, float* mean, float* rstd,
                                   long long M, int H, float eps, float q_scale,
                                   const float* rope_cos, const float* rope_sin, int S, int St, void* stream) {
    if (M <= 0 || H <= 0 || (ld % 8) || (ldo % 8) || ld < 2 * H * 64 || ldo < 2 * H * 64) return VT_ERR_BAD_SHAPE;
    if ((rope_cos == nullptr) != (rope_sin == nullptr)) return VT_ERR_BAD_SHAPE;
    if (rope_cos != nullptr && (S <= 0 || St < 0 || St > S || (M % S))) return VT_ERR_BAD_SHAPE;
    if ((((uintptr_t)rope_cos) | ((uintptr_t)rope_sin)) & 15) return VT_ERR_BAD_ALIGN;
    if ((((uintptr_t)qkv) | ((uintptr_t)out) | ((uintptr_t)gq) | ((uintptr_t)bq) | ((uintptr_t)gk) | ((uintptr_t)bk)) & 15)
        return VT_ERR_BAD_ALIGN;
    const long long threads = M * 2 * H * 8;
    const long long blocks = (threads + 255) / 256;
    if (blocks > 0x7fffffffLL) return VT_ERR_BAD_SHAPE;
    hipLaunchKernelGGL(qk_layernorm_fwd_kernel, dim3((unsigned)blocks), dim3(256), 0, (hipStream_t)stream,
                       (const bf16_t*)qkv, ld, (bf16_t*)out, ldo, (const bf16_t*)gq, (const bf16_t*)bq,
                       (const bf16_t*)gk, (const bf16_t*)bk, mean, rstd, M, H, eps, q_scale, rope_cos, rope_sin,
                       S > 0 ? S : 1, St);
    return hipGetLastError() == hipSuccess ? VT_OK : VT_ERR_LAUNCH;
}

extern "C" int vt_qk_layernorm_bwd(const float* dq_hat, int lddq, const void* dk_hat, int lddk, const void* qkv, int ld,
                                   const float* mean, const float* rstd, const void* gq, const void* gk,
                                   void* dqkv, int ldd, long long M, int H,
                                   const float* rope_cos, const float* rope_sin, int S, int St, void* stream) {
    if (M <= 0 || H <= 0 || (ld % 8) || (ldd % 8) || (lddq % 4) || (lddk % 8)) return VT_ERR_BAD_SHAPE;
    if ((rope_cos == nullptr) != (rope_sin == nullptr)) return VT_ERR_BAD_SHAPE;
    if (rope_cos != nullptr && (S <= 0 || St < 0 || St > S || (M % S))) return VT_ERR_BAD_SHAPE;
    if ((((uintptr_t)rope_cos) | ((uintptr_t)rope_sin)) & 15) return VT_ERR_BAD_ALIGN;
    if ((((uintptr_t)qkv) | ((uintptr_t)dqkv) | ((uintptr_t)dq_hat) | ((uintptr_t)dk_hat) | ((uintptr_t)gq) | ((uintptr_t)gk)) & 15)
        return VT_ERR_BAD_ALIGN;
    const long long threads = M * 2 * H * 8;
    const long long blocks = (threads + 255) / 256;
    if (blocks > 0x7fffffffLL) return VT_ERR_BAD_SHAPE;
    hipLaunchKernelGGL(qk_layernorm_bwd_kernel, dim3((unsigned)blocks), dim3(256), 0, (hipStream_t)stream,
                       dq_hat, lddq, (const bf16_t*)dk_hat, lddk, (const bf16_t*)qkv, ld, mean, rstd,
                       (const bf16_t*)gq, (const bf16_t*)gk, (bf16_t*)dqkv, ldd, M, H, rope_cos, rope_sin, S > 0 ? S : 1, St);
    return hipGetLastError() == hipSuccess ? VT_OK : VT_ERR_LAUNCH;
}
```

videotuna-dev_amd/engine.py:

```python
from __future__ import annotations

from types import SimpleNamespace
from typing import List, Optional

import torch

from . import ops
from .lora import TARGETS
from .ops import BF16, EPI_BIAS, EPI_BIAS_GELU, EPI_DGELU, EPI_GATED_RES

EXT = 64
Q_PRESCALE = 1.4426950408889634 / 8.0


def _lin(mod):
    base = getattr(mod, "base_layer", mod)
    return base.weight, base.bias


def _ext_widths(model):
    st = model.lora
    return (st.ext_qkv, st.ext_o) if st is not None else (EXT, EXT)


# ... 95 lines not shown
    if (model._packed is None or (ft is not None and model._packed.ft_version != ft.version)
            or model._packed.ext != _ext_widths(model) or model._packed.ff != _ff_lora(model)
            or model._packed.dora != (_dora(model) is not None)):
        model._packed = pack(model)
    P = model._packed
    st = model.lora
    if st is not None and P.lora_version != st.version:
        d, r, rp, eq, eo = model.inner_dim, st.r, st.rp, st.ext_qkv, st.ext_o
        ff1, ff2, ef = P.ff
        if st.wide:
            pack_b = lambda b, w, ld, n: ops.lora_pack_b_wide(b, w, ld, 1, n, r, rp, ef, st.scaling)
            pack_bt = lambda b, w, ld, n: ops.lora_pack_bt_wide(b, w, ld, 1, n, r, rp, ef, st.scaling)
        else:
            pack_b = lambda b, w, ld, n: ops.lora_pack_b(b, w, ld, 1, n, r, st.scaling)
            pack_bt = lambda b, w, ld, n: ops.lora_pack_bt(b, w, ld, 1, n, r, st.scaling)
        for i, L in enumerate(P.layers):
            if ff1:
                dff, b1 = L.w1.shape[0], st.view(st.flat, i, "B", 4)
                pack_b(b1, L.w1[:, d:], d + ef, dff)
                pack_bt(b1, L.w1_t[d:], dff, dff)
            if ff2:
                dff, b2 = L.w2_t.shape[0], st.view(st.flat, i, "B", 5)
                pack_b(b2, L.w2[:, dff:], dff + ef, d)
                pack_bt(b2, L.w2_bt, d, d)
                L.w2_t[:, d:d + r].copy_(ops.transpose(st.view(st.flat_bf16, i, "A", 5)))
            if st.wide:
                ops.lora_pack_b_wide(st.b_qkv(st.flat, i), L.w_qkv[:, d:], d + eq, 3, d, r, rp, eq, st.scaling)
                ops.lora_pack_bt_wide(st.b_qkv(st.flat, i), L.w_qkv_t[d:], 3 * d, 3, d, r, rp, eq, st.scaling)
                ops.lora_pack_b_wide(st.b_out(st.flat, i), L.w_o[:, d:], d + eo, 1, d, r, rp, eo, st.scaling)
                ops.lora_pack_bt_wide(st.b_out(st.flat, i), L.w_o_t[d:], d, 1, d, r, rp, eo, st.scaling)
                continue
            ops.lora_pack_b(st.b_qkv(st.flat, i), L.w_qkv[:, d:], d + eq, 3, d, r, st.scaling)
            ops.lora_pack_bt(st.b_qkv(st.flat, i), L.w_qkv_t[d:], 3 * d, 3, d, r, st.scaling)
            ops.lora_pack_b(st.b_out(st.flat, i), L.w_o[:, d:], d + eo, 1, d, r, st.scaling)
            ops.lora_pack_bt(st.b_out(st.flat, i), L.w_o_t[d:], d, 1, d, r, st.scaling)
        if P.dora:
            for i, L in enumerate(P.layers):
                _dora_refresh(model, st, i, L, P.ff)
        P.lora_version = st.version
    return P


def _dora_fold(st, w0, a, b, n, mag, c, w_fwd, wt_base, wt_ext, not_adapted=()):
    K = w0.shape[1]
    ops.dora_norm(w0, a, b, n, st.r, st.scaling, c, mag=mag)
    for rows in not_adapted:
        c[rows].fill_(1.0)
    ops.dora_scale(w0, w_fwd[:, :K], c)
    ops.dora_scale(w_fwd[:, K:], w_fwd[:, K:], c)
    ops.dora_transpose_scale(w0, wt_base, c)
    ops.dora_scale(wt_ext, wt_ext, c, by_col=True)


def _dora_refresh(model, st, i, L, ff):
    d, bf = model.inner_dim, st.flat_bf16
    ff1, ff2, _ = ff
    blk = model.transformer_blocks[i]
    qkv = [t in st.targets for t in ("to_q", "to_k", "to_v")]
    if any(qkv):
        _dora_fold(st, L.w_qkv0, st.a_qkv(bf, i), st.b_qkv(bf, i), 3, st.mag_qkv(st.flat, i), L.c_qkv, L.w_qkv, L.w_qkv_t[:d], L.w_qkv_t[d:],
                   [slice(j * d, (j + 1) * d) for j in range(3) if not qkv[j]])
    if "to_out.0" in st.targets:
        _dora_fold(st, _lin(blk.attn1.to_out[0])[0], st.a_out(bf, i), st.b_out(bf, i), 1, st.view(st.flat, i, "M", 3), L.c_o, L.w_o,
                   L.w_o_t[:d], L.w_o_t[d:])
    if ff1:
        _dora_fold(st, _lin(blk.ff.net[0].proj)[0], st.view(bf, i, "A", 4), st.view(bf, i, "B", 4), 1, st.view(st.flat, i, "M", 4), L.c_1,
                   L.w1, L.w1_t[:d], L.w1_t[d:])
    if ff2:
        _dora_fold(st, _lin(blk.ff.net[2])[0], st.view(bf, i, "A", 5), st.view(bf, i, "B", 5), 1, st.view(st.flat, i, "M", 5), L.c_2,
                   L.w2, L.w2_t[:, :d], L.w2_bt)


def _lora_db(st, tn, big, small, gB, P, c=None):
    out = gB if c is None else st.dora_scratch(gB.numel()).view(gB.shape)
    for j in range(gB.shape[0] // P):
        tn(big[:, j * P:], small[:, j * st.rp:], st.r, out[j * P:], st.r, 1, st.scaling, P)
    if c is not None:
        ops.dora_db_add(gB, out, c)


def _dora_dm(st, i, j, g, y, bias, n=1):
    N = g.shape[1]
    sums = st.dora_scratch(2 * N)
    ops.group_colsum(g, sums[:N], y=y, out2=sums[N:])
    d = N // n
    for k in range(n):
        if TARGETS[j + k] in st.targets:
            cols = slice(k * d, (k + 1) * d)
            ops.dora_dm(sums[:N][cols], sums[N:][cols], None if bias is None else bias[cols], st.view(st.flat, i, "M", j + k),
                        st.view(st.grad, i, "M", j + k))


def lora_dropout_seed(model):
    st = model.lora
    if st is None or not getattr(st, "p", 0.0) or not model.training:
        return None
    seed = getattr(model, "lora_dropout_seed", None)
    if seed is None:
        seed = int(torch.randint(0, 2 ** 62, (1,)).item())
    model.last_lora_dropout_seed = int(seed)
    return float(st.p), int(seed)


def _lora_proj(st, i, proj, buf):
    if proj == "qkv":
        return 3, st.a_qkv(buf, i), st.ext_qkv, 4 * i
    if proj == "ff1":
        return 1, st.view(buf, i, "A", 4), st.ext_ff, 4 * st.L + 2 * i
    if proj == "ff2":
        return 1, st.view(buf, i, "A", 5), st.ext_ff, 4 * st.L + 2 * i + 1
    return 1, st.a_out(buf, i), st.ext_o, 4 * i + 3


def _narrow_calls(n, r):
    return [(0, n)] if n * r <= 16 else [(j, 1) for j in range(n)]


def _lora_down(st, i, proj, x, d, drop=None):
    n, a, ext, site = _lora_proj(st, i, proj, st.flat_bf16)
    r, rp = st.r, st.rp
    if st.wide:
        if drop is None:
            ops.lora_down_wide(x, a, n, r, rp, ext, x[:, d:], d)
        elif ops.lora_down_wide_drop_fits(n, rp):
            ops.lora_down_wide_drop(x, a, n, r, rp, ext, x[:, d:], d, *drop, site)
        else:
            for j in range(n):
                ops.lora_down_wide_drop(x, a[j * r:(j + 1) * r], 1, r, rp, rp if j < n - 1 else ext - j * rp, x[:, d + j * rp:], d,
                                        *drop, site + j)
        return
    for j, nj in _narrow_calls(n, r):
        zc = EXT - 16 - j * r if j + nj == n else 0
        if drop is None:
            ops.lora_down(x, a[j * r:(j + nj) * r], nj * r, x[:, d + j * r:], d, zero_cols=zc)
        else:
            ops.lora_down_drop(x, a[j * r:(j + nj) * r], nj * r, nj, x[:, d + j * r:], d, *drop, site + j, zero_cols=zc)


def _lora_da(st, i, proj, x, dxe, d, drop=None, dt0=None):
    n, ga, _, site = _lora_proj(st, i, proj, st.grad)
    r = st.r
    for j, nj in ([(j, 1) for j in range(n)] if st.wide else _narrow_calls(n, r)):
        dt, g = (dxe[:, d + j * st.rp:] if dt0 is None else dt0[:, j * st.rp:]), ga[j * r:(j + nj) * r]
        if st.wide and drop is None:
            ops.lora_tn_wide(x, dt, r, g, 1, d, 1.0, d)
        elif st.wide:
            ops.lora_tn_wide_drop(x, dt, r, g, 1, d, 1.0, d, *drop, site + j)
        elif drop is None:
            ops.skinny_tn(x, dt, nj * r, g, 1, d, 1.0, d)
        else:
            ops.skinny_tn_drop(x, dt, nj * r, nj, g, 1, d, 1.0, d, *drop, site + j)


def _lora_dx(st, i, proj, dxe, d, drop=None):
    n, a, _, site = _lora_proj(st, i, proj, st.flat_bf16)
    r = st.r
    if st.wide:
        if drop is None:
            ops.lora_up_add_wide(dxe, dxe[:, d:], a, n, r, st.rp, d)
        else:
            ops.lora_up_add_wide_drop(dxe, dxe[:, d:], a, n, r, st.rp, d, *drop, site)
        return
    for j, nj in _narrow_calls(n, r):
        if drop is None:
            ops.lora_up_add(dxe, dxe[:, d + j * r:], a[j * r:(j + nj) * r], nj * r, d)
        else:
            ops.lora_up_add_drop(dxe, dxe[:, d + j * r:], a[j * r:(j + nj) * r], nj * r, nj, d, *drop, site + j)


def _lora_dx_dgelu(st, i, du, dt, u, K, drop):
    _, a, _, site = _lora_proj(st, i, "ff2", st.flat_bf16)
    if st.wide:
        ops.lora_up_add_wide_dgelu_drop(du, dt, a, 1, st.r, st.rp, u, K, *drop, site)
    else:
        ops.lora_up_add_dgelu_drop(du, dt, a, st.r, 1, u, K, *drop, site)


def _lora_down_qkv(x1, st, i, d, drop=None):
    _lora_down(st, i, "qkv", x1, d, drop)


def _lora_qkv_input_grads(x1, dx1, st, i, d, need_dx=True, drop=None):
    _lora_da(st, i, "qkv", x1, dx1, d, drop)
    if need_dx:
        _lora_dx(st, i, "qkv", dx1, d, drop)


def _mod(mod: torch.Tensor, idx: int, d: int):
    o = idx * 6 * d
    v = lambda k: mod[:, o + k * d:]
    return SimpleNamespace(shift_vid=v(0), scale_vid=v(1), gate_vid=v(2), shift_txt=v(3), scale_txt=v(4), gate_txt=v(5),
                           bs=mod.stride(0))


def saved_bytes_per_block(model, M: int) -> int:
    d = model.inner_dim
    ext2 = sum(_ext_widths(model)) if model.lora is not None else 0
    cols = 2 * d + ext2 + 3 * d + 2 * d + d + model.config.ff_mult * d + d
    if getattr(model, "fullft", None) is not None:
        cols += d + model.config.ff_mult * d + 2 * d
    ff1, ff2, ef = _ff_lora(model)
    cols += (d + ef if ff1 else 0) + (model.config.ff_mult * d + ef if ff2 else 0)
    dora = _dora(model)
    if dora is not None:
        cols += (d if "to_out.0" in dora.targets else 0) + (d if ff2 else 0)
    return M * cols * 2


def _use_recompute(model, dims) -> bool:
    import os
    mode = os.environ.get("VT355_RECOMPUTE") or getattr(model, "recompute", "never")
    if mode == "always":
        return True
    if mode != "auto":
        return False
    need = saved_bytes_per_block(model, dims[-1]) * model.config.num_layers
    free, _ = torch.cuda.mem_get_info()
    return need > 0.6 * free


def block_forward(model, i: int, h, mod, dims, rope, save: bool, scratch, drop=None):
    c = model.config
    P = packed(model)
    st = model.lora
    ft = getattr(model, "fullft", None)
    d, H = model.inner_dim, c.num_attention_heads
    B, Fr, C, Hh, Ww, S, St, Sv, M = dims
    dev = h.device
    eq, eo = _ext_widths(model)
    KEq, KEo = (d + eq, d + eo) if st is not None else (d, d)
    E = lambda *s, dt=BF16: torch.empty(*s, dtype=dt, device=dev)
    xg, gbuf = scratch.xg, scratch.gbuf
    Lw = P.layers[i]
    m1, m2 = _mod(mod, 2 * i, d), _mod(mod, 2 * i + 1, d)
    a = SimpleNamespace(h_in=h)
    x1 = E(M, d + eq)
    a.mean1, a.rstd1 = E(M, dt=torch.float32), E(M, dt=torch.float32)
    ops.ln_modulate_fwd(h, x1, Lw.n1g, Lw.n1b, (m1.shift_txt, m1.scale_txt, m1.shift_vid, m1.scale_vid, m1.bs),
                        a.mean1, a.rstd1, d, S, St, c.norm_eps)
    if st is not None:
        _lora_down(st, i, "qkv", x1, d, drop)
    qkv = E(M, 3 * d)
    ops.gemm(x1, Lw.w_qkv, qkv, Lw.b_qkv, K=KEq)
    qkh = E(M, 2 * d)
    a.qmean, a.qrstd = E(M, 2 * H, dt=torch.float32), E(M, 2 * H, dt=torch.float32)
    ops.qk_layernorm_fwd(qkv, qkh, Lw.gq, Lw.bq, Lw.gk, Lw.bk, a.qmean, a.qrstd, H, 1e-6, q_scale=Q_PRESCALE, rope=rope)
    o = E(M, d + eo)
    lse = E(B, H, S, dt=torch.float32)
    qk3, qkv3, o3 = qkh.view(B, S, 2 * d), qkv.view(B, S, 3 * d), o.view(B, S, d + eo)
    ops.attn_fwd(qk3[:, :, :d], qk3[:, :, d:], qkv3[:, :, 2 * d:], o3[:, :, :d], lse, B, H, S, q_prescaled=True)
    if st is not None:
        _lora_down(st, i, "out", o, d, drop)
    h1 = E(M, d)
    dora = _dora(model)
    ao = E(M, d) if (save and (ft is not None or (dora is not None and "to_out.0" in dora.targets))) else None
    ops.gemm(o, Lw.w_o, h1, Lw.b_o, epilogue=EPI_GATED_RES, residual=h, gate_txt=m1.gate_txt, gate_vid=m1.gate_vid,
             gate_bstride=m1.bs, S=S, St=St, K=KEo, pre_act_out=ao)
    a.mean2, a.rstd2 = E(M, dt=torch.float32), E(M, dt=torch.float32)
    keep_ff = save and ft is not None
    ff1, ff2, ef = _ff_lora(model)
    dff = c.ff_mult * d
    x2 = E(M, d + ef if ff1 else d) if (keep_ff or (save and ff1)) else xg
    gact = E(M, dff + ef if ff2 else dff) if (keep_ff or (save and ff2)) else gbuf
    ops.ln_modulate_fwd(h1, x2, Lw.n2g, Lw.n2b, (m2.shift_txt, m2.scale_txt, m2.shift_vid, m2.scale_vid, m2.bs),
                        a.mean2, a.rstd2, d, S, St, c.norm_eps)
    if ff1:
        _lora_down(st, i, "ff1", x2, d, drop)
    u = E(M, dff) if save else gbuf.new_empty(M, dff)
    ops.gemm(x2, Lw.w1, gact, Lw.b1, epilogue=EPI_BIAS_GELU, pre_act_out=u, K=d + ef if ff1 else None)
    if ff2:
        _lora_down(st, i, "ff2", gact, dff, drop)
    h2 = E(M, d)
    fo = E(M, d) if (keep_ff or (save and dora is not None and ff2)) else None
    ops.gemm(gact, Lw.w2, h2, Lw.b2, epilogue=EPI_GATED_RES, residual=h1, gate_txt=m2.gate_txt, gate_vid=m2.gate_vid,
             gate_bstride=m2.bs, S=S, St=St, pre_act_out=fo, K=dff + ef if ff2 else None)
    if save:
        a.x1, a.qkv, a.qkh, a.o, a.lse, a.h1, a.u = x1, qkv, qkh, o, lse, h1, u
        a.x2, a.g, a.ao, a.fo = (x2, gact, ao, fo) if ft is not None else (x2 if ff1 else None, gact if ff2 else None, ao, fo)
    return h2, a


def run_forward(model, x, text, t, save: bool, rope=None):
    c = model.config
    P = packed(model)
    st = model.lora
    d, H, L = model.inner_dim, c.num_attention_heads, c.num_layers
    B, Fr, C, Hh, Ww = x.shape
    p = c.patch_size
    Sv, St = Fr * (Hh // p) * (Ww // p), text.shape[1]
    S = St + Sv
    M = B * S
    dev = x.device
    ft = getattr(model, "fullft", None)
    E = lambda *s, dt=BF16: torch.empty(*s, dtype=dt, device=dev)

    te = c.time_embed_dim
    tsin = E(B, d); ops.timestep_embedding(t, tsin, c.flip_sin_to_cos, float(c.freq_shift))
    e1_pre = E(B, te); ops.gemm(tsin, P.t1_w, e1_pre, P.t1_b)
    e1 = E(B, te); ops.silu(e1_pre, e1)
    emb_pre = E(B, te); ops.gemm(e1, P.t2_w, emb_pre, P.t2_b)
    emb = E(B, te); ops.silu(emb_pre, emb)
    mod = E(B, P.w_ada.shape[0], dt=torch.float32); ops.gemm(emb, P.w_ada, mod, P.b_ada)

    h = E(M, d)
    patches = E(B * Sv, C * p * p); ops.patchify(x, patches, p)
    pos = model.pos_table(Fr, Hh, Ww, dev)
    pos_txt = model.patch_embed.pos_embedding[0, :St] if c.use_learned_positional_embeddings else None
    for b in range(B):
        if pos is not None:
            ops.gemm(patches[b * Sv:(b + 1) * Sv], P.patch_w, h[b * S + St:(b + 1) * S], P.patch_b,
                     epilogue=EPI_GATED_RES, residual=pos)
        else:
            ops.gemm(patches[b * Sv:(b + 1) * Sv], P.patch_w, h[b * S + St:(b + 1) * S], P.patch_b)
        if pos_txt is not None:
            ops.gemm(text[b], P.text_w, h[b * S:b * S + St], P.text_b, epilogue=EPI_GATED_RES, residual=pos_txt)
        else:
            ops.gemm(text[b], P.text_w, h[b * S:b * S + St], P.text_b)
    if rope is not None:
        rope = (rope[0], rope[1], S, St)

    dims = (B, Fr, C, Hh, Ww, S, St, Sv, M)
    ff1, ff2, ef = _ff_lora(model)
    scratch = SimpleNamespace(xg=E(M, d + ef if ff1 else d),
                              gbuf=E(M, c.ff_mult * d + (ef if ff2 else 0)))
    recompute = save and _use_recompute(model, dims)
    drop = lora_dropout_seed(model)
    saved: List[SimpleNamespace] = []
    for i in range(L):
        h2, a = block_forward(model, i, h, mod, dims, rope, save and not recompute, scratch, drop)
        if save:
            saved.append(a)
        h = h2

    mo = 2 * L * 6 * d
    f_shift, f_scale = mod[:, mo:], mod[:, mo + d:]
    y1 = E(B * Sv, d); y2 = E(B * Sv, d)
    fm1, fr1 = E(B * Sv, dt=torch.float32), E(B * Sv, dt=torch.float32)
    fm2, fr2 = E(B * Sv, dt=torch.float32), E(B * Sv, dt=torch.float32)
    for b in range(B):
        rows = slice(b * Sv, (b + 1) * Sv)
        ops.ln_modulate_fwd(h[b * S + St:(b + 1) * S], y1[rows], model.norm_final.weight, model.norm_final.bias, None,
                            fm1[rows], fr1[rows], d, Sv, 0, c.norm_eps)
    ops.ln_modulate_fwd(y1, y2, model.norm_out.norm.weight, model.norm_out.norm.bias,
                        (f_shift, f_scale, f_shift, f_scale, mod.stride(0)), fm2, fr2, d, Sv, 0, c.norm_eps)
    tok = E(B * Sv, P.proj_w.shape[0])
    ops.gemm(y2, P.proj_w, tok, P.proj_b)
    out = E(B, Fr, c.out_channels, Hh, Ww)
    ops.unpatchify(tok, out, p)
    ctx = None
    if save:
        ctx = SimpleNamespace(blocks=saved, mod=mod, h_last=h, y1=y1, fm1=fm1, fr1=fr1, fm2=fm2, fr2=fr2,
                              dims=dims, f_scale=f_scale, rope=rope, recompute=recompute, scratch=scratch if recompute else None,
                              lora_drop=drop)
        if ft is not None:
            ctx.y2, ctx.tsin, ctx.e1_pre, ctx.e1, ctx.emb_pre, ctx.se, ctx.patches, ctx.text = y2, tsin, e1_pre, e1, emb_pre, emb, patches, text
    return out, ctx


def run_backward(model, ctx, dout: torch.Tensor):
    c = model.config
    P = packed(model)
    st = model.lora
    d, H, L = model.inner_dim, c.num_attention_heads, c.num_layers
    B, Fr, C, Hh, Ww, S, St, Sv, M = ctx.dims
    p = c.patch_size
    dev = dout.device
    eq, eo = st.ext_qkv, st.ext_o
    tn = ops.lora_tn_wide if st.wide else ops.skinny_tn
    E = lambda *s, dt=BF16: torch.empty(*s, dtype=dt, device=dev)
    mod = ctx.mod
    drop = ctx.lora_drop
    dora = _dora(model) is not None

    dtok = E(B * Sv, c.out_channels * p * p); ops.patchify(dout, dtok, p)
    dy2 = E(B * Sv, d); ops.gemm(dtok, P.proj_w_t, dy2, None)
    dy1 = E(B * Sv, d)
    ops.ln_modulate_bwd(dy2, ctx.y1, ctx.fm2, ctx.fr2, model.norm_out.norm.weight, (ctx.f_scale, ctx.f_scale, mod.stride(0)),
                        None, dy1, d, Sv, 0)
    dh = torch.zeros(M, d, dtype=BF16, device=dev)
    for b in range(B):
        rows = slice(b * Sv, (b + 1) * Sv)
        ops.ln_modulate_bwd(dy1[rows], ctx.h_last[b * S + St:(b + 1) * S], ctx.fm1[rows], ctx.fr1[rows],
                            model.norm_final.weight, None, None, dh[b * S + St:(b + 1) * S], d, Sv, 0)

    ff1, ff2, ef = _ff_lora(model)
    dff = c.ff_mult * d
    tg = E(M, d)
    tgf = E(M, d + ef) if ff2 else tg
    du = E(M, dff)
    dx2 = E(M, d + ef) if ff1 else E(M, d)
    dh1 = E(M, d)
    dO = E(M, d + eo)
    dq = E(B, S, d, dt=torch.float32)
    dkh = E(M, d)
    dqkv = E(M, 3 * d)
    dx1 = E(M, d + eq)
    delta = E(B * H * S, dt=torch.float32)
    chain_ws = ops.attn_bwd_chain_workspace(B, H, S, dev)
    dh_in = E(M, d)
    for i in reversed(range(L)):
        Lw, a = P.layers[i], ctx.blocks[i]
        if ctx.recompute:
            _, a = block_forward(model, i, a.h_in, mod, ctx.dims, ctx.rope, True, ctx.scratch, drop)
        m1, m2 = _mod(mod, 2 * i, d), _mod(mod, 2 * i + 1, d)
        ops.gate_mul(dh, tgf, m2.gate_txt, m2.gate_vid, m2.bs, d, S, St)
        if ff2:
            ops.gemm(tgf, Lw.w2_bt, tgf[:, d:], None, K=d)
            _lora_db(st, tn, tgf, a.g[:, dff:], st.view(st.grad, i, "B", 5), d, Lw.c_2 if dora else None)
            if dora:
                _dora_dm(st, i, 5, tgf[:, :d], a.fo, Lw.b2)
            _lora_da(st, i, "ff2", a.g, None, dff, drop, dt0=tgf[:, d:])
            if drop is None:
                ops.gemm(tgf, Lw.w2_t, du, None, epilogue=EPI_DGELU, pre_act_in=a.u, K=d + ef)
            else:
                ops.gemm(tgf, Lw.w2_t, du, None, epilogue=EPI_DGELU, pre_act_in=a.u, K=d)
                _lora_dx_dgelu(st, i, du, tgf[:, d:], a.u, dff, drop)
        else:
            ops.gemm(tg, Lw.w2_t, du, None, epilogue=EPI_DGELU, pre_act_in=a.u)
        ops.gemm(du, Lw.w1_t, dx2, None)
        if ff1:
            _lora_db(st, tn, du, a.x2[:, d:], st.view(st.grad, i, "B", 4), dff, Lw.c_1 if dora else None)
            if dora:
                _dora_dm(st, i, 4, du, a.u, Lw.b1)
            _lora_da(st, i, "ff1", a.x2, dx2, d, drop)
            _lora_dx(st, i, "ff1", dx2, d, drop)
        ops.ln_modulate_bwd(dx2, a.h1, a.mean2, a.rstd2, Lw.n2g, (m2.scale_txt, m2.scale_vid, m2.bs), dh, dh1, d, S, St)
        ops.gate_mul(dh1, tg, m1.gate_txt, m1.gate_vid, m1.bs, d, S, St)
        ops.gemm(tg, Lw.w_o_t, dO, None)
        out_adapted = dora and "to_out.0" in st.targets
        _lora_db(st, tn, tg, a.o[:, d:], st.b_out(st.grad, i), d, Lw.c_o if out_adapted else None)
        if out_adapted:
            _dora_dm(st, i, 3, tg, a.ao, Lw.b_o)
        _lora_da(st, i, "out", a.o, dO, d, drop)
        _lora_dx(st, i, "out", dO, d, drop)
        dq.zero_()
        qk3, qkv3 = a.qkh.view(B, S, 2 * d), a.qkv.view(B, S, 3 * d)
        ops.attn_bwd(qk3[:, :, :d], qk3[:, :, d:], qkv3[:, :, 2 * d:], a.o.view(B, S, d + eo)[:, :, :d],
                     dO.view(B, S, d + eo)[:, :, :d], a.lse, delta, dq, dkh.view(B, S, d),
                     dqkv.view(B, S, 3 * d)[:, :, 2 * d:], B, H, S, q_prescaled=True, chain_ws=chain_ws)
        ops.qk_layernorm_bwd(dq.view(M, d), dkh, a.qkv, a.qmean, a.qrstd, Lw.gq, Lw.gk, dqkv, H, rope=ctx.rope)
        if i > 0:
            ops.gemm(dqkv, Lw.w_qkv_t, dx1, None)
        else:
            ops.gemm(dqkv, Lw.w_qkv_t[d:], dx1[:, d:], None)
        qkv_adapted = dora and any(t in st.targets for t in TARGETS[:3])
        _lora_db(st, tn, dqkv, a.x1[:, d:], st.b_qkv(st.grad, i), d, Lw.c_qkv if qkv_adapted else None)
        if qkv_adapted:
            _dora_dm(st, i, 0, dqkv, a.qkv, Lw.b_qkv, n=3)
        _lora_da(st, i, "qkv", a.x1, dx1, d, drop)
        if i > 0:
            _lora_dx(st, i, "qkv", dx1, d, drop)
            ops.ln_modulate_bwd(dx1, a.h_in, a.mean1, a.rstd1, Lw.n1g, (m1.scale_txt, m1.scale_vid, m1.bs), dh1, dh_in,
                                d, S, St)
            dh, dh_in = dh_in, dh
        ctx.blocks[i] = None
    return None


class _DiTFn(torch.autograd.Function):
    @staticmethod
    def forward(ctx, anchor, model, x, text, t, rope):
        out, saved = run_forward(model, x, text, t, save=True, rope=rope)
        ctx.model, ctx.saved = model, saved
        return out

    @staticmethod
    def backward(ctx, dout):
        if getattr(ctx.model, "fullft", None) is not None:
            from .engine_fullft import run_backward_fullft
            run_backward_fullft(ctx.model, ctx.saved, dout.contiguous(), ctx.model.fullft.on_grads_ready)
        else:
            run_backward(ctx.model, ctx.saved, dout.contiguous())
        ctx.saved = None
        return None, None, None, None, None, None


def _rope_tables(model, image_rotary_emb, Sv: int, dev):
    if image_rotary_emb is None:
        return None
    cos, sin = image_rotary_emb
    out = []
    for tb in (cos, sin):
        if tuple(tb.shape) != (Sv, model.config.attention_head_dim):
            raise ValueError(f"image_rotary_emb tables must be [{Sv}, {model.config.attention_head_dim}], got {tuple(tb.shape)}")
        out.append(tb.detach().to(device=dev, dtype=torch.float32).contiguous())
    return out[0], out[1]


def dit_apply(model, hidden_states, encoder_hidden_states, timestep, image_rotary_emb=None):
    x = hidden_states
    if x.dtype != BF16:
        raise TypeError(f"hidden_states must be bf16 (model dtype), got {x.dtype}")
    x = x.contiguous()
    text = encoder_hidden_states
    if text.dtype == torch.float32:
        tb = torch.empty(text.shape, dtype=BF16, device=text.device)
        ops.cast_f32_bf16(text.contiguous(), tb)
        text = tb
    text = text.contiguous()
    if timestep.dim() == 0:
        timestep = timestep[None].expand(x.shape[0])
    t = timestep.to(torch.int64).contiguous()
    st = model.lora
    need_grad = torch.is_grad_enabled() and ((st is not None and any(p.requires_grad for p in st.params))
                                             or getattr(model, "fullft", None) is not None)
    p = model.config.patch_size
    rope = _rope_tables(model, image_rotary_emb, x.shape[1] * (x.shape[3] // p) * (x.shape[4] // p), x.device)
    if not need_grad:
        out, _ = run_forward(model, x, text, t, save=False, rope=rope)
        return out
    anchor = torch.zeros(1, device=x.device, requires_grad=True)
    return _DiTFn.apply(anchor, model, x, text, t, rope)
```

videotuna-dev_amd/ops.py:

```python
from __future__ import annotations

import math
import os
from typing import Optional

import torch

from ._lib import check, load_library

BF16 = torch.bfloat16
EPI_BIAS, EPI_BIAS_GELU, EPI_GATED_RES, EPI_DGELU = 0, 1, 2, 3


def _stream() -> int:
    return torch.cuda.current_stream().cuda_stream


_PROFILE = {"on": False, "events": {}, "work": {}}
_PROFILED = ("attn_fwd", "attn_bwd", "conv", "conv_dw")


def profile_reset(on: bool):
    _PROFILE["on"] = on
    if on:
# ... 226 lines not shown

def _cl_check(t, nm):
    ld = t.stride(3)
    N, T, H, W, _ = t.shape
    if t.stride(2) != W * ld or t.stride(1) != H * W * ld or t.stride(0) != T * H * W * ld:
        raise ValueError(f"{nm}: positions must be uniformly strided (channels-last, only the channel axis may be a slice)")


def causal_conv3d(x, wk, bias, y, residual=None):
    _req(x, BF16, "x", 5); _req(y, BF16, "y", 5); _req(wk, BF16, "wk", 2)
    N, T, H, W, Cin = x.shape
    Cout = y.shape[4]
    if tuple(y.shape[:4]) != (N, T, H, W) or tuple(wk.shape) != (Cout, 27 * Cin) or not wk.is_contiguous():
        raise ValueError(f"shape mismatch: x {tuple(x.shape)} wk {tuple(wk.shape)} y {tuple(y.shape)}")
    _cl_check(x, "x"); _cl_check(y, "y")
    if residual is not None:
        _req(residual, BF16, "residual", 5); _cl_check(residual, "residual")
        if tuple(residual.shape) != tuple(y.shape):
            raise ValueError("residual must have the shape of y")
    check(load_library().vt_causal_conv3d_cl(x.data_ptr(), x.stride(3), wk.data_ptr(), _p(bias), _p(residual),
                                             0 if residual is None else residual.stride(3), y.data_ptr(), y.stride(3),
                                             N, T, H, W, Cin, Cout, _stream()), "vt_causal_conv3d_cl")
    return y


def pack_conv_in8_weight(w: torch.Tensor) -> torch.Tensor:
    if w.dim() != 5 or tuple(w.shape[2:]) != (3, 3, 3) or w.shape[1] > 8:
        raise ValueError(f"expected a [Cout, Cin<=8, 3, 3, 3] weight, got {tuple(w.shape)}")
    out = torch.zeros(w.shape[0], 32, 8, dtype=w.dtype, device=w.device)
    out[:, :27, :w.shape[1]] = w.permute(0, 2, 3, 4, 1).reshape(w.shape[0], 27, w.shape[1])
    return out.reshape(w.shape[0], 256)


def causal_conv3d_in8(x, wk, bias, y):
    _req(x, BF16, "x", 5); _req(y, BF16, "y", 5); _req(wk, BF16, "wk", 2)
    N, T, H, W, C8 = x.shape
    Cout = y.shape[4]
    if C8 != 8 or not x.is_contiguous() or tuple(y.shape[:4]) != (N, T, H, W) or tuple(wk.shape) != (Cout, 256) or not wk.is_contiguous():
        raise ValueError(f"shape mismatch: x {tuple(x.shape)} wk {tuple(wk.shape)} y {tuple(y.shape)}")
    _cl_check(y, "y")
    check(load_library().vt_causal_conv3d_in8_cl(x.data_ptr(), wk.data_ptr(), _p(bias), y.data_ptr(), y.stride(3), N, T, H, W, Cout,
                                                 _stream()), "vt_causal_conv3d_in8_cl")
    return y


def downsample_conv2d(x, wk, bias, y):
    _req(x, BF16, "x", 5); _req(y, BF16, "y", 5); _req(wk, BF16, "wk", 2)
    N, T, H, W, Cin = x.shape
    Cout = y.shape[4]
    if tuple(y.shape[:4]) != (N, T, H // 2, W // 2) or tuple(wk.shape) != (Cout, 9 * Cin) or not wk.is_contiguous():
        raise ValueError(f"shape mismatch: x {tuple(x.shape)} wk {tuple(wk.shape)} y {tuple(y.shape)}")
    _cl_check(x, "x"); _cl_check(y, "y")
    check(load_library().vt_downsample_conv2d_cl(x.data_ptr(), x.stride(3), wk.data_ptr(), _p(bias), y.data_ptr(), y.stride(3),
                                                 N, T, H, W, Cin, Cout, _stream()), "vt_downsample_conv2d_cl")
    return y


def temporal_pool_frames(T: int, keep_first: bool) -> int:
    return 1 + (T - 1) // 2 if keep_first else T // 2


def temporal_pool(x, y, keep_first: bool = True):
    _req(x, BF16, "x", 5); _req(y, BF16, "y", 5)
    N, T, H, W, C = x.shape
    To = temporal_pool_frames(T, keep_first)
    if tuple(y.shape) != (N, To, H, W, C) or To < 1:
        raise ValueError(f"y must be {(N, To, H, W, C)}, got {tuple(y.shape)}")
    _cl_check(x, "x"); _cl_check(y, "y")
    check(load_library().vt_temporal_pool_cl(x.data_ptr(), x.stride(3), y.data_ptr(), y.stride(3), N, T, H * W, C, int(keep_first),
                                             _stream()), "vt_temporal_pool_cl")
    return y


def rmsnorm(x, w, y, eps: float = 1e-6):
    _req(x, BF16, "x", 2); _req(y, BF16, "y", 2); _req(w, BF16, "w", 1)
    check(load_library().vt_rmsnorm_bf16(x.data_ptr(), x.stride(0), w.data_ptr(), y.data_ptr(), y.stride(0), x.shape[0], x.shape[1],
                                         eps, _stream()), "vt_rmsnorm_bf16")


def gated_gelu(u, y):
    _req(u, BF16, "u", 2); _req(y, BF16, "y", 2)
    check(load_library().vt_gated_gelu_bf16(u.data_ptr(), u.stride(0), y.data_ptr(), y.stride(0), u.shape[0], y.shape[1], _stream()),
          "vt_gated_gelu_bf16")


def attn_bwd_chain_workspace(B: int, H: int, S: int, device) -> Optional[torch.Tensor]:
    if _SIDE_STREAMS["n"] > 0 or _CHAIN_STATE["disabled"]:
        return None
    n = int(load_library().vt_attn_bwd_chain_ws_bytes(B, H, S))
    if n <= 0:
        return None
    key = str(device)
    ws = _CHAIN_WS.get(key)
    if ws is None or ws.numel() < n:
        old = ws
        ws = _CHAIN_WS[key] = torch.empty(n, dtype=torch.uint8, device=device)
        ws[:256].zero_()
        if old is not None:
            ws[64:256].copy_(old[64:256])
    return ws


_CHAIN_WS = {}
_SIDE_STREAMS = {"n": 0}
_CHAIN_STATE = {"disabled": False, "redone": 0, "verify": __import__("os").environ.get("VT355_CHAIN_VERIFY", "launch")}


def attn_bwd_chain_redone() -> int:
    return _CHAIN_STATE["redone"]


def declare_side_stream(active: bool):
    _SIDE_STREAMS["n"] = max(0, _SIDE_STREAMS["n"] + (1 if active else -1))


def chain_guard(device) -> Optional[torch.Tensor]:
    ws = _CHAIN_WS.get(str(device))
    return None if ws is None else ws[64:68].view(torch.int32)


def attn_bwd_chain_errors() -> int:
    return sum(int(ws[64:68].view(torch.int32).item()) for ws in _CHAIN_WS.values())


def attn_bwd_chain_errors_clear():
    for ws in _CHAIN_WS.values():
        ws[64:256].zero_()


def conv_set_tile(mode: int = 0):
    check(load_library().vt_conv_set_tile(mode), "vt_conv_set_tile")


def gemm_set_tile(mode: int = 0):
    check(load_library().vt_gemm_set_tile(mode), "vt_gemm_set_tile")


def gemm_kernel(M: int, N: int, K: int) -> int:
    k = load_library().vt_gemm_bf16_kernel(M, N, K)
    if k < 0:
        check(k, "vt_gemm_bf16_kernel")
    return k


def attn_bwd_set_chain(chain_len: int = 0, slots: int = 0):
    check(load_library().vt_attn_bwd_set_chain(chain_len, slots), "vt_attn_bwd_set_chain")


def attn_bwd_chain_error(chain_ws: torch.Tensor) -> int:
    return int(chain_ws[32:36].view(torch.int32).item())


def attn_bwd(q, k, v, o, do, lse2, delta_ws, dq_f32, dk, dv, B: int, H: int, S: int, scale: Optional[float] = None,
             q_prescaled: bool = False, chain_ws: Optional[torch.Tensor] = None, _entry=None):
    scale = 1.0 / math.sqrt(64) if scale is None else scale
    for n, t in (("q", q), ("k", k), ("v", v), ("o", o), ("do", do), ("dk", dk), ("dv", dv)):
        _req(t, BF16, n, 3)
    _req(dq_f32, torch.float32, "dq_f32", 3)
    lib = load_library()

    def launch(ws, fn=None):
        check((fn or lib.vt_attn_bwd_hd64)(q.data_ptr(), k.data_ptr(), v.data_ptr(), o.data_ptr(), do.data_ptr(),
                               lse2.data_ptr(), delta_ws.data_ptr(), dq_f32.data_ptr(), dk.data_ptr(), dv.data_ptr(),
                               B, H, S,
                               q.stride(1), k.stride(1), v.stride(1), o.stride(1), do.stride(1),
                               dq_f32.stride(1), dk.stride(1), dv.stride(1),
                               q.stride(0), k.stride(0), v.stride(0), o.stride(0), do.stride(0),
                               dq_f32.stride(0), dk.stride(0), dv.stride(0), scale, int(q_prescaled),
                               None if ws is None else ws.data_ptr(), 0 if ws is None else ws.numel(),
                               _stream()),
          "vt_attn_bwd_hd64")
    with _timed("attn_bwd"):
        launch(chain_ws, _entry)
    if chain_ws is not None and _CHAIN_STATE["verify"] == "launch" and attn_bwd_chain_error(chain_ws) != 0:
        import warnings
        _CHAIN_STATE["disabled"] = True
        _CHAIN_STATE["redone"] += 1
        warnings.warn("vt_attn_bwd_hd64: a dQ hand-off wait timed out (the persistent workgroups were not all resident: another stream or a "
                      "profiler shared the CUs); the launch was redone with plain atomics and the hand-off chains are switched off for the rest "
                      "of this process (VT_BWD_CHAIN=1 avoids them from the start; ops.declare_side_stream(True) announces a concurrent stream)")
        dq_f32.zero_()
        launch(None)
        chain_ws[32:36].zero_()
        chain_ws[64:68].zero_()


def ln_modulate_fwd(x, y, gamma, beta, mod, mean, rstd, D: int, S: int, St: int, eps: float):
    _req(x, BF16, "x", 2); _req(y, BF16, "y", 2)
    m = (None, None, None, None, 0) if mod is None else mod
    lib = load_library()
    with _timed_hbm("ln_modulate_fwd", x.shape[0], 4.0 * x.shape[0] * D):
        check(lib.vt_ln_modulate_fwd(x.data_ptr(), x.stride(0), y.data_ptr(), y.stride(0), _p(gamma), _p(beta),
                                     _p(m[0]), _p(m[1]), _p(m[2]), _p(m[3]), m[4], _p(mean), _p(rstd),
                                     x.shape[0], D, S, St, eps, _stream()), "vt_ln_modulate_fwd")


def ln_modulate_bwd(dy, x, mean, rstd, gamma, scales, dres, dx, D: int, S: int, St: int):
    _req(dy, BF16, "dy", 2); _req(x, BF16, "x", 2); _req(dx, BF16, "dx", 2)
    sc = (None, None, 0) if scales is None else scales
    lib = load_library()
    with _timed_hbm("ln_modulate_bwd", x.shape[0], (6.0 if dres is None else 8.0) * x.shape[0] * D):
        check(lib.vt_ln_modulate_bwd(dy.data_ptr(), dy.stride(0), x.data_ptr(), x.stride(0), mean.data_ptr(), rstd.data_ptr(),
                                     _p(gamma), _p(sc[0]), _p(sc[1]), sc[2], _p(dres), 0 if dres is None else dres.stride(0),
                                     dx.data_ptr(), dx.stride(0), x.shape[0], D, S, St, _stream()), "vt_ln_modulate_bwd")


def qk_layernorm_fwd(qkv, out, gq, bq, gk, bk, mean, rstd, H: int, eps: float, q_scale: float = 1.0, rope=None):
    _req(qkv, BF16, "qkv", 2); _req(out, BF16, "out", 2)
    lib = load_library()
    rc, rsn, S, St = _rope_args(rope, qkv.shape[0])
    with _timed_hbm("qk_layernorm_fwd", qkv.shape[0], 8.0 * qkv.shape[0] * H * 64):
        check(lib.vt_qk_layernorm_fwd(qkv.data_ptr(), qkv.stride(0), out.data_ptr(), out.stride(0), gq.data_ptr(), bq.data_ptr(),
                                      gk.data_ptr(), bk.data_ptr(), mean.data_ptr(), rstd.data_ptr(), qkv.shape[0], H, eps,
                                      q_scale, rc, rsn, S, St, _stream()), "vt_qk_layernorm_fwd")


def qk_layernorm_bwd(dq_hat_f32, dk_hat, qkv, mean, rstd, gq, gk, dqkv, H: int, rope=None):
    _req(dq_hat_f32, torch.float32, "dq_hat", 2); _req(dk_hat, BF16, "dk_hat", 2)
    lib = load_library()
    rc, rsn, S, St = _rope_args(rope, qkv.shape[0])
    with _timed_hbm("qk_layernorm_bwd", qkv.shape[0], 14.0 * qkv.shape[0] * H * 64):
        check(lib.vt_qk_layernorm_bwd(dq_hat_f32.data_ptr(), dq_hat_f32.stride(0), dk_hat.data_ptr(), dk_hat.stride(0),
                                      qkv.data_ptr(), qkv.stride(0), mean.data_ptr(), rstd.data_ptr(), gq.data_ptr(), gk.data_ptr(),
                                      dqkv.data_ptr(), dqkv.stride(0), qkv.shape[0], H, rc, rsn, S, St, _stream()),
              "vt_qk_layernorm_bwd")


def gate_mul(x, y, g_txt, g_vid, bstride: int, D: int, S: int, St: int):
    _req(x, BF16, "x", 2); _req(y, BF16, "y", 2)
    lib = load_library()
    check(lib.vt_gate_mul(x.data_ptr(), x.stride(0), y.data_ptr(), y.stride(0), g_txt.data_ptr(), g_vid.data_ptr(), bstride,
                          x.shape[0], D, S, St, _stream()), "vt_gate_mul")


def silu(x, y):
    _req(x, BF16, "x"); _req(y, BF16, "y")
    check(load_library().vt_silu_bf16(x.data_ptr(), y.data_ptr(), x.numel(), _stream()), "vt_silu_bf16")


def cast_f32_bf16(x, y):
    _req(x, torch.float32, "x"); _req(y, BF16, "y")
    check(load_library().vt_cast_f32_bf16(x.data_ptr(), y.data_ptr(), x.numel(), _stream()), "vt_cast_f32_bf16")


def timestep_embedding(t, out, flip: bool = True, freq_shift: float = 0.0):
    _req(t, torch.int64, "t", 1); _req(out, BF16, "out", 2)
    check(load_library().vt_timestep_embedding(t.data_ptr(), out.data_ptr(), out.shape[0], out.shape[1], int(flip),
                                               freq_shift, _stream()), "vt_timestep_embedding")


def patchify(img, tok, P: int):
    _req(img, BF16, "img", 5); _req(tok, BF16, "tok", 2)
    B, F, C, H, W = img.shape
    check(load_library().vt_patchify(img.data_ptr(), tok.data_ptr(), B, F, C, H, W, P, tok.stride(0), _stream()), "vt_patchify")


def unpatchify(tok, img, P: int):
    _req(img, BF16, "img", 5); _req(tok, BF16, "tok", 2)
    B, F, C, H, W = img.shape
    check(load_library().vt_unpatchify(tok.data_ptr(), img.data_ptr(), B, F, C, H, W, P, tok.stride(0), _stream()),
          "vt_unpatchify")


def add_noise(x0, noise, sa, sb, noisy):
    _req(x0, torch.float32, "x0"); _req(noise, torch.float32, "noise"); _req(noisy, BF16, "noisy")
    B = x0.shape[0]
    check(load_library().vt_add_noise(x0.data_ptr(), noise.data_ptr(), sa.data_ptr(), sb.data_ptr(), noisy.data_ptr(),
                                      x0.numel() // B, B, _stream()), "vt_add_noise")


def diffusion_loss(vpred, noisy, x0, sa, sb, w, loss, partials, dvpred, grad_scale: float = 1.0):
    _req(vpred, BF16, "vpred"); _req(noisy, BF16, "noisy"); _req(x0, torch.float32, "x0")
    B = x0.shape[0]
    check(load_library().vt_diffusion_loss(vpred.data_ptr(), noisy.data_ptr(), x0.data_ptr(), sa.data_ptr(), sb.data_ptr(),
                                           w.data_ptr(), loss.data_ptr(), partials.data_ptr(), _p(dvpred),
                                           x0.numel() // B, B, grad_scale, _stream()), "vt_diffusion_loss")


def diffusion_loss_bwd(vpred, noisy, x0, sa, sb, w, grad_out, dvpred):
    _req(grad_out, torch.float32, "grad_out")
    B = x0.shape[0]
    check(load_library().vt_diffusion_loss_bwd(vpred.data_ptr(), noisy.data_ptr(), x0.data_ptr(), sa.data_ptr(), sb.data_ptr(),
                                               w.data_ptr(), grad_out.data_ptr(), dvpred.data_ptr(), x0.numel() // B, B,
                                               _stream()), "vt_diffusion_loss_bwd")


def adamw(p, g, m, v, p_bf16, lr, beta1, beta2, eps, wd, step: int, grad_scale: float = 1.0, guard: Optional[torch.Tensor] = None,
          clip_coef: Optional[torch.Tensor] = None, clip_value: float = 0.0):
    for n, t in (("p", p), ("g", g), ("m", m), ("v", v)):
        _req(t, torch.float32, n)
    if guard is not None:
        _req(guard, torch.int32, "guard")
    with _timed_hbm("adamw", p.numel(), (28.0 + (2.0 if p_bf16 is not None else 0.0)) * p.numel()):
        if clip_coef is None and not clip_value > 0.0:
            check(load_library().vt_adamw(p.data_ptr(), g.data_ptr(), m.data_ptr(), v.data_ptr(), _p(p_bf16), p.numel(),
                                          lr, beta1, beta2, eps, wd, step, grad_scale, _p(guard), _stream()), "vt_adamw")
        else:
            if clip_coef is not None:
                _req(clip_coef, torch.float32, "clip_coef")
            check(load_library().vt_adamw_clip(p.data_ptr(), g.data_ptr(), m.data_ptr(), v.data_ptr(), _p(p_bf16), p.numel(),
                                               lr, beta1, beta2, eps, wd, step, grad_scale, _p(guard), _p(clip_coef),
                                               float(clip_value), _stream()), "vt_adamw_clip")


def grad_sqnorm_partials() -> int:
    return int(load_library().vt_grad_sqnorm_partials())


def grad_sqnorm(g, partials, slot: int = 0):
    _req(g, torch.float32, "g"); _req(partials, torch.float32, "partials")
    if partials.numel() < (slot + 1) * grad_sqnorm_partials():
        raise ValueError("partials holds fewer than slot + 1 slots")
    check(load_library().vt_grad_sqnorm(g.data_ptr(), g.numel(), partials.data_ptr(), slot, _stream()), "vt_grad_sqnorm")


def clip_finalize(partials, nslots: int, grad_scale: float, max_norm: float, record):
    _req(partials, torch.float32, "partials"); _req(record, torch.float32, "record")
    if partials.numel() < nslots * grad_sqnorm_partials() or record.numel() < 2:
        raise ValueError("partials / record too small")
    check(load_library().vt_clip_finalize(partials.data_ptr(), nslots, float(grad_scale), float(max_norm), record.data_ptr(),
                                          _stream()), "vt_clip_finalize")


def lora_down(x, a, R: int, t_out, K: int, zero_cols: int = 48):
    _req(x, BF16, "x", 2); _req(a, BF16, "a", 2); _req(t_out, BF16, "t", 2)
    check(load_library().vt_lora_down(x.data_ptr(), x.stride(0), a.data_ptr(), a.stride(0), R, t_out.data_ptr(),
                                      t_out.stride(0), x.shape[0], K, zero_cols, _stream()), "vt_lora_down")


_SKINNY_WS = {}


def _skinny_ws(lib, big, P: int, use_workspace: bool):
    if not use_workspace:
        return None
    need = lib.vt_skinny_tn_workspace_bytes(P) // 4
    key = big.device
    if key not in _SKINNY_WS or _SKINNY_WS[key].numel() < need:
        _SKINNY_WS[key] = torch.empty(need, dtype=torch.float32, device=big.device)
    return _SKINNY_WS[key]


def skinny_tn(big, small, R: int, out, osp: int, osr: int, alpha: float, P: int, use_workspace: bool = False):
    _req(big, BF16, "big", 2); _req(small, BF16, "small", 2); _req(out, torch.float32, "out")
    lib = load_library()
    ws = _skinny_ws(lib, big, P, use_workspace)
    check(lib.vt_skinny_tn(big.data_ptr(), big.stride(0), small.data_ptr(), small.stride(0), R, out.data_ptr(),
                           osp, osr, alpha, big.shape[0], P, _p(ws), _stream()), "vt_skinny_tn")


def lora_up_add(dx, dt, a, R: int, K: int):
    _req(dx, BF16, "dx", 2); _req(dt, BF16, "dt", 2); _req(a, BF16, "a", 2)
    check(load_library().vt_lora_up_add(dx.data_ptr(), dx.stride(0), dt.data_ptr(), dt.stride(0), a.data_ptr(), a.stride(0),
                                        R, dx.shape[0], K, _stream()), "vt_lora_up_add")


def lora_pack_b(bcat_f32, wext, ldw: int, n_adapters: int, d_out: int, r: int, scale: float):
    check(load_library().vt_lora_pack_b(bcat_f32.data_ptr(), wext.data_ptr(), ldw, n_adapters, d_out, r, scale, _stream()),
          "vt_lora_pack_b")


def lora_pack_bt(bcat_f32, wtext, ldwt: int, n_adapters: int, d_out: int, r: int, scale: float):
    check(load_library().vt_lora_pack_bt(bcat_f32.data_ptr(), wtext.data_ptr(), ldwt, n_adapters, d_out, r, scale, _stream()),
          "vt_lora_pack_bt")


def lora_down_wide(x, a, n_adapters: int, r: int, rp: int, ext: int, t_out, K: int):
    _req(x, BF16, "x", 2); _req(a, BF16, "a", 2); _req(t_out, BF16, "t", 2)
    check(load_library().vt_lora_down_wide(x.data_ptr(), x.stride(0), a.data_ptr(), a.stride(0), n_adapters, r, rp, ext,
                                           t_out.data_ptr(), t_out.stride(0), x.shape[0], K, _stream()), "vt_lora_down_wide")


def lora_tn_wide(big, small, R: int, out, osp: int, osr: int, alpha: float, P: int):
    _req(big, BF16, "big", 2); _req(small, BF16, "small", 2); _req(out, torch.float32, "out")
    check(load_library().vt_lora_tn_wide(big.data_ptr(), big.stride(0), small.data_ptr(), small.stride(0), R, out.data_ptr(),
                                         osp, osr, alpha, big.shape[0], P, _stream()), "vt_lora_tn_wide")


def lora_up_add_wide(dx, dt, a, n_adapters: int, r: int, rp: int, K: int):
    _req(dx, BF16, "dx", 2); _req(dt, BF16, "dt", 2); _req(a, BF16, "a", 2)
    check(load_library().vt_lora_up_add_wide(dx.data_ptr(), dx.stride(0), dt.data_ptr(), dt.stride(0), a.data_ptr(), a.stride(0),
                                             n_adapters, r, rp, dx.shape[0], K, _stream()), "vt_lora_up_add_wide")


def lora_pack_b_wide(bcat_f32, wext, ldw: int, n_adapters: int, d_out: int, r: int, rp: int, ext: int, scale: float):
    check(load_library().vt_lora_pack_b_wide(bcat_f32.data_ptr(), wext.data_ptr(), ldw, n_adapters, d_out, r, rp, ext, scale,
                                             _stream()), "vt_lora_pack_b_wide")


def lora_pack_bt_wide(bcat_f32, wtext, ldwt: int, n_adapters: int, d_out: int, r: int, rp: int, ext: int, scale: float):
    check(load_library().vt_lora_pack_bt_wide(bcat_f32.data_ptr(), wtext.data_ptr(), ldwt, n_adapters, d_out, r, rp, ext, scale,
                                              _stream()), "vt_lora_pack_bt_wide")


_U64 = 0xFFFFFFFFFFFFFFFF


def lora_down_drop(x, a, R: int, n_adapters: int, t_out, K: int, p: float, seed: int, site0: int, zero_cols: int = 48):
    _req(x, BF16, "x", 2); _req(a, BF16, "a", 2); _req(t_out, BF16, "t", 2)
    check(load_library().vt_lora_down_drop(x.data_ptr(), x.stride(0), a.data_ptr(), a.stride(0), R, n_adapters, t_out.data_ptr(),
                                           t_out.stride(0), x.shape[0], K, zero_cols, float(p), int(seed) & _U64, site0, _stream()),
          "vt_lora_down_drop")


def skinny_tn_drop(big, small, R: int, n_adapters: int, out, osp: int, osr: int, alpha: float, P: int, p: float, seed: int, site0: int,
                   use_workspace: bool = False):
    _req(big, BF16, "big", 2); _req(small, BF16, "small", 2); _req(out, torch.float32, "out")
    lib = load_library()
    ws = _skinny_ws(lib, big, P, use_workspace)
    check(lib.vt_skinny_tn_drop(big.data_ptr(), big.stride(0), small.data_ptr(), small.stride(0), R, n_adapters, out.data_ptr(),
                                osp, osr, alpha, big.shape[0], P, _p(ws), float(p), int(seed) & _U64, site0, _stream()),
          "vt_skinny_tn_drop")


def lora_up_add_drop(dx, dt, a, R: int, n_adapters: int, K: int, p: float, seed: int, site0: int):
    _req(dx, BF16, "dx", 2); _req(dt, BF16, "dt", 2); _req(a, BF16, "a", 2)
    check(load_library().vt_lora_up_add_drop(dx.data_ptr(), dx.stride(0), dt.data_ptr(), dt.stride(0), a.data_ptr(), a.stride(0),
                                             R, n_adapters, dx.shape[0], K, float(p), int(seed) & _U64, site0, _stream()),
          "vt_lora_up_add_drop")


def lora_down_wide_drop_fits(n_adapters: int, rp: int) -> bool:
    return bool(load_library().vt_lora_down_wide_drop_fits(n_adapters, rp))


def lora_down_wide_drop(x, a, n_adapters: int, r: int, rp: int, ext: int, t_out, K: int, p: float, seed: int, site0: int):
    _req(x, BF16, "x", 2); _req(a, BF16, "a", 2); _req(t_out, BF16, "t", 2)
    check(load_library().vt_lora_down_wide_drop(x.data_ptr(), x.stride(0), a.data_ptr(), a.stride(0), n_adapters, r, rp, ext,
                                                t_out.data_ptr(), t_out.stride(0), x.shape[0], K, float(p), int(seed) & _U64, site0,
                                                _stream()), "vt_lora_down_wide_drop")


def lora_tn_wide_drop(big, small, R: int, out, osp: int, osr: int, alpha: float, P: int, p: float, seed: int, site: int):
    _req(big, BF16, "big", 2); _req(small, BF16, "small", 2); _req(out, torch.float32, "out")
    check(load_library().vt_lora_tn_wide_drop(big.data_ptr(), big.stride(0), small.data_ptr(), small.stride(0), R, out.data_ptr(),
                                              osp, osr, alpha, big.shape[0], P, float(p), int(seed) & _U64, site, _stream()),
          "vt_lora_tn_wide_drop")


def lora_up_add_wide_drop(dx, dt, a, n_adapters: int, r: int, rp: int, K: int, p: float, seed: int, site0: int):
    _req(dx, BF16, "dx", 2); _req(dt, BF16, "dt", 2); _req(a, BF16, "a", 2)
    check(load_library().vt_lora_up_add_wide_drop(dx.data_ptr(), dx.stride(0), dt.data_ptr(), dt.stride(0), a.data_ptr(), a.stride(0),
                                                  n_adapters, r, rp, dx.shape[0], K, float(p), int(seed) & _U64, site0, _stream()),
          "vt_lora_up_add_wide_drop")


def _req_preact(u, dx, K: int, dt=None, a=None, rows: int = 0, cols: int = 0):
    _req(u, BF16, "u", 2)
    if u.shape[0] != dx.shape[0] or u.shape[1] < K or dx.shape[1] < K:
        raise ValueError(f"u {tuple(u.shape)} / dx {tuple(dx.shape)}: expected {dx.shape[0]} rows of at least K = {K} columns")
    if dt is not None and (dt.shape[0] != dx.shape[0] or dt.shape[1] < cols or a.shape[0] < rows or a.shape[1] < K):
        raise ValueError(f"dt {tuple(dt.shape)} / a {tuple(a.shape)}: expected dt [{dx.shape[0]}, >= {cols}] and a [>= {rows}, >= {K}]")


def lora_up_add_dgelu_drop(dx, dt, a, R: int, n_adapters: int, u, K: int, p: float, seed: int, site0: int):
    _req(dx, BF16, "dx", 2); _req(dt, BF16, "dt", 2); _req(a, BF16, "a", 2); _req_preact(u, dx, K, dt, a, R, R)
    check(load_library().vt_lora_up_add_dgelu_drop(dx.data_ptr(), dx.stride(0), dt.data_ptr(), dt.stride(0), a.data_ptr(), a.stride(0),
                                                   R, n_adapters, u.data_ptr(), u.stride(0), dx.shape[0], K, float(p), int(seed) & _U64,
                                                   site0, _stream()), "vt_lora_up_add_dgelu_drop")


def lora_up_add_wide_dgelu_drop(dx, dt, a, n_adapters: int, r: int, rp: int, u, K: int, p: float, seed: int, site0: int):
    _req(dx, BF16, "dx", 2); _req(dt, BF16, "dt", 2); _req(a, BF16, "a", 2)
    _req_preact(u, dx, K, dt, a, n_adapters * r, n_adapters * rp)
    check(load_library().vt_lora_up_add_wide_dgelu_drop(dx.data_ptr(), dx.stride(0), dt.data_ptr(), dt.stride(0), a.data_ptr(),
                                                        a.stride(0), n_adapters, r, rp, u.data_ptr(), u.stride(0), dx.shape[0], K,
                                                        float(p), int(seed) & _U64, site0, _stream()),
          "vt_lora_up_add_wide_dgelu_drop")


def dora_norm(w, a, b, n_adapters: int, r: int, scale: float, out, mag=None):
    _req(w, BF16, "w", 2); _req(a, BF16, "a", 2); _req(b, BF16, "b", 2); _req(out, torch.float32, "out", 1)
    N, K = w.shape
    if mag is not None:
        _req(mag, torch.float32, "mag", 1)
    if (N % n_adapters or a.shape[0] < n_adapters * r or a.shape[1] < K or b.shape[0] != N or b.shape[1] != r or not b.is_contiguous()
            or out.numel() < N or (mag is not None and mag.numel() < N)):
        raise ValueError(f"dora_norm: w {tuple(w.shape)}, a {tuple(a.shape)}, b {tuple(b.shape)}, out {tuple(out.shape)} do not fit "
                         f"{n_adapters} adapter(s) of rank {r}")
    check(load_library().vt_dora_norm(w.data_ptr(), w.stride(0), a.data_ptr(), a.stride(0), b.data_ptr(), n_adapters, N // n_adapters, r, K,
                                      float(scale), _p(mag), out.data_ptr(), _stream()), "vt_dora_norm")


def dora_scale(src, dst, c, by_col: bool = False):
    _req(src, BF16, "src", 2); _req(dst, BF16, "dst", 2); _req(c, torch.float32, "c", 1)
    rows, cols = src.shape
    if tuple(dst.shape) != (rows, cols) or c.numel() < (cols if by_col else rows):
        raise ValueError(f"dora_scale: src {tuple(src.shape)}, dst {tuple(dst.shape)}, c {tuple(c.shape)}")
    check(load_library().vt_dora_scale(src.data_ptr(), src.stride(0), dst.data_ptr(), dst.stride(0), c.data_ptr(), rows, cols, int(by_col),
                                       _stream()), "vt_dora_scale")


def dora_transpose_scale(src, dst, c):
    _req(src, BF16, "src", 2); _req(dst, BF16, "dst", 2); _req(c, torch.float32, "c", 1)
    rows, cols = src.shape
    if tuple(dst.shape) != (cols, rows) or c.numel() < rows:
        raise ValueError(f"dora_transpose_scale: src {tuple(src.shape)}, dst {tuple(dst.shape)}, c {tuple(c.shape)}")
    check(load_library().vt_dora_transpose_scale(src.data_ptr(), src.stride(0), dst.data_ptr(), dst.stride(0), c.data_ptr(), rows, cols,
                                                 _stream()), "vt_dora_transpose_scale")


def dora_db_add(g, s, c):
    _req(g, torch.float32, "g", 2); _req(s, torch.float32, "s", 2); _req(c, torch.float32, "c", 1)
    if tuple(g.shape) != tuple(s.shape) or not g.is_contiguous() or not s.is_contiguous() or c.numel() < g.shape[0]:
        raise ValueError(f"dora_db_add: g {tuple(g.shape)}, s {tuple(s.shape)}, c {tuple(c.shape)}")
    check(load_library().vt_dora_db_add(g.data_ptr(), s.data_ptr(), c.data_ptr(), g.shape[0], g.shape[1], _stream()), "vt_dora_db_add")

# ... 593 lines not shown
```

Before: 2.820 samples/s.

## Fuse gate_mul into LN backward and attention delta into LoRA up-add

The LayerNorm-modulate backward kernel can now also write the gated gradient for the next stage, which removes the separate gate_mul passes over the residual gradient. The LoRA dX up-add for to_out now computes the attention backward delta (the per-head rowsum of O·dO) while the freshly updated dO is still in registers. A new attention-backward entry point then skips its own delta kernel. Together these cut several full-activation HBM read/write passes per layer, at the cost of extra register use in the fused kernels. Both paths are on by default and can be disabled with an environment variable.

After: 2.835 samples/s (median of 6 runs). About the same (+0.5%).

```diff
diff --git a/include/vt355.h b/include/vt355.h
--- a/include/vt355.h
+++ b/include/vt355.h
@@ -85,6 +85,14 @@
                      long long q_bs, long long k_bs, long long v_bs, long long o_bs, long long do_bs,
                      long long dq_bs, long long dk_bs, long long dv_bs,
                      float softmax_scale, int q_prescaled, void* chain_ws, long long chain_ws_bytes, void* stream);
+int vt_attn_bwd_hd64_delta(const void* q, const void* k, const void* v, const void* o, const void* dout,
+                           const float* lse2, float* delta_ws, float* dq_f32, void* dk, void* dv,
+                           int B, int H, int S,
+                           long long q_rs, long long k_rs, long long v_rs, long long o_rs, long long do_rs,
+                           long long dq_rs, long long dk_rs, long long dv_rs,
+                           long long q_bs, long long k_bs, long long v_bs, long long o_bs, long long do_bs,
+                           long long dq_bs, long long dk_bs, long long dv_bs,
+                           float softmax_scale, int q_prescaled, void* chain_ws, long long chain_ws_bytes, void* stream);
 long long vt_attn_bwd_chain_ws_bytes(int B, int H, int S);
 int vt_attn_bwd_set_chain(int chain_len, int slots);
 
@@ -96,6 +104,11 @@
                        const void* gamma, const float* scale_txt, const float* scale_vid, int mod_bstride,
                        const void* dres, int lddres, void* dx, int lddx,
                        int M, int D, int S, int St, void* stream);
+int vt_ln_modulate_bwd_gate(const void* dy, int lddy, const void* x, int ldx, const float* mean, const float* rstd,
+                            const void* gamma, const float* scale_txt, const float* scale_vid, int mod_bstride,
+                            const void* dres, int lddres, void* dx, int lddx, int M, int D, int S, int St,
+                            const float* gate_txt, const float* gate_vid, int gate_bstride, void* gated_out, int ldg,
+                            void* stream);
 
 int vt_qk_layernorm_fwd(const void* qkv, int ld, void* out, int ldo, const void* gq, const void* bq,
                         const void* gk, const void* bk, float* mean, float* rstd,
@@ -142,6 +155,8 @@
 long long vt_skinny_tn_workspace_bytes(int P);
 int vt_lora_up_add(void* dX, int ldx, const void* dT, int ldt, const void* A, int lda, int R, long long M, int K,
                    void* stream);
+int vt_lora_up_add_delta(void* dX, int ldx, const void* dT, int ldt, const void* A, int lda, int R, long long M, int K,
+                         const void* O, int ldo, float* delta, int S, void* stream);
 int vt_lora_pack_b(const float* Bcat, void* Wext, int ldw, int n_adapters, int d_out, int r, float scale, void* stream);
 int vt_lora_pack_bt(const float* Bcat, void* WText, int ldwt, int n_adapters, int d_out, int r, float scale, void* stream);
 
diff --git a/videotuna-dev_amd/_lib.py b/videotuna-dev_amd/_lib.py
--- a/videotuna-dev_amd/_lib.py
+++ b/videotuna-dev_amd/_lib.py
@@ -46,10 +46,14 @@
     "vt_gated_gelu_bf16": [_vp, _ll, _vp, _ll, _ll, _i, _vp],
     "vt_attn_bwd_hd64": [_vp, _vp, _vp, _vp, _vp, _fp, _fp, _fp, _vp, _vp, _i, _i, _i,
                          _ll, _ll, _ll, _ll, _ll, _ll, _ll, _ll, _ll, _ll, _ll, _ll, _ll, _ll, _ll, _ll, _f, _i, _vp, _ll, _vp],
+    "vt_attn_bwd_hd64_delta": [_vp, _vp, _vp, _vp, _vp, _fp, _fp, _fp, _vp, _vp, _i, _i, _i,
+                               _ll, _ll, _ll, _ll, _ll, _ll, _ll, _ll, _ll, _ll, _ll, _ll, _ll, _ll, _ll, _ll, _f, _i, _vp, _ll, _vp],
     "vt_attn_bwd_chain_ws_bytes": [_i, _i, _i],
     "vt_attn_bwd_set_chain": [_i, _i],
     "vt_ln_modulate_fwd": [_vp, _i, _vp, _i, _vp, _vp, _fp, _fp, _fp, _fp, _i, _fp, _fp, _i, _i, _i, _i, _f, _vp],
     "vt_ln_modulate_bwd": [_vp, _i, _vp, _i, _fp, _fp, _vp, _fp, _fp, _i, _vp, _i, _vp, _i, _i, _i, _i, _i, _vp],
+    "vt_ln_modulate_bwd_gate": [_vp, _i, _vp, _i, _fp, _fp, _vp, _fp, _fp, _i, _vp, _i, _vp, _i, _i, _i, _i, _i,
+                                _fp, _fp, _i, _vp, _i, _vp],
     "vt_qk_layernorm_fwd": [_vp, _i, _vp, _i, _vp, _vp, _vp, _vp, _fp, _fp, _ll, _i, _f, _f, _fp, _fp, _i, _i, _vp],
     "vt_qk_layernorm_bwd": [_fp, _i, _vp, _i, _vp, _i, _fp, _fp, _vp, _vp, _vp, _i, _ll, _i, _fp, _fp, _i, _i, _vp],
     "vt_gate_mul": [_vp, _i, _vp, _i, _fp, _fp, _i, _ll, _i, _i, _i, _vp],
@@ -70,6 +74,7 @@
     "vt_skinny_tn": [_vp, _i, _vp, _i, _i, _fp, _ll, _ll, _f, _ll, _i, _fp, _vp],
     "vt_skinny_tn_workspace_bytes": [_i],
     "vt_lora_up_add": [_vp, _i, _vp, _i, _vp, _i, _i, _ll, _i, _vp],
+    "vt_lora_up_add_delta": [_vp, _i, _vp, _i, _vp, _i, _i, _ll, _i, _vp, _i, _fp, _i, _vp],
     "vt_lora_pack_b": [_fp, _vp, _i, _i, _i, _i, _f, _vp],
     "vt_lora_pack_bt": [_fp, _vp, _i, _i, _i, _i, _f, _vp],
     "vt_lora_down_wide": [_vp, _i, _vp, _i, _i, _i, _i, _i, _vp, _i, _ll, _i, _vp],
diff --git a/videotuna-dev_amd/csrc/attn_bwd.hip b/videotuna-dev_amd/csrc/attn_bwd.hip
--- a/videotuna-dev_amd/csrc/attn_bwd.hip
+++ b/videotuna-dev_amd/csrc/attn_bwd.hip
@@ -588,7 +588,7 @@
     return VT_OK;
 }
 
-extern "C" int BWD_ENTRY(const void* q, const void* k, const void* v, const void* o, const void* dout,
+static int bwd_launch(const void* q, const void* k, const void* v, const void* o, const void* dout,
                                 const float* lse2, float* delta_ws, float* dq_f32, void* dk, void* dv,
                                 int B, int H, int S,
                                 long long q_rs, long long k_rs, long long v_rs, long long o_rs, long long do_rs,
@@ -596,7 +596,7 @@
                                 long long q_bs, long long k_bs, long long v_bs, long long o_bs, long long do_bs,
                                 long long dq_bs, long long dk_bs, long long dv_bs,
                                 float softmax_scale, int q_prescaled, void* chain_ws, long long chain_ws_bytes,
-                                void* stream) {
+                                int have_delta, void* stream) {
     if (B <= 0 || H <= 0 || S <= 0) return VT_ERR_BAD_SHAPE;
     if ((long long)S * dq_rs * 4 >= 0x7fffffffLL) return VT_ERR_BAD_SHAPE;
     if ((q_rs % 8) || (k_rs % 8) || (v_rs % 8) || (o_rs % 8) || (do_rs % 8) || (dk_rs % 4) || (dv_rs % 4)) return VT_ERR_BAD_SHAPE;
@@ -607,7 +607,7 @@
     if ((long long)S * q_rs * 2 >= lim || (long long)S * k_rs * 2 >= lim || (long long)S * v_rs * 2 >= lim ||
         (long long)S * do_rs * 2 >= lim) return VT_ERR_BAD_SHAPE;
     hipStream_t st = (hipStream_t)stream;
-    {
+    if (!have_delta) {
         const long long total = (long long)B * S * H * 8;
         const int blocks = (int)((total + 255) / 256);
         hipLaunchKernelGGL(DELTA_KERNEL, dim3(blocks), dim3(256), 0, st, (const bf16_t*)o, (const bf16_t*)dout,
@@ -647,6 +647,20 @@
     return hipGetLastError() == hipSuccess ? VT_OK : VT_ERR_LAUNCH;
 }
 
+#define BWD_ARGS_DECL const void* q, const void* k, const void* v, const void* o, const void* dout, \
+                      const float* lse2, float* delta_ws, float* dq_f32, void* dk, void* dv, int B, int H, int S, \
+                      long long q_rs, long long k_rs, long long v_rs, long long o_rs, long long do_rs, \
+                      long long dq_rs, long long dk_rs, long long dv_rs, \
+                      long long q_bs, long long k_bs, long long v_bs, long long o_bs, long long do_bs, \
+                      long long dq_bs, long long dk_bs, long long dv_bs, \
+                      float softmax_scale, int q_prescaled, void* chain_ws, long long chain_ws_bytes, void* stream
+#define BWD_ARGS q, k, v, o, dout, lse2, delta_ws, dq_f32, dk, dv, B, H, S, q_rs, k_rs, v_rs, o_rs, do_rs, dq_rs, dk_rs, dv_rs, \
+                 q_bs, k_bs, v_bs, o_bs, do_bs, dq_bs, dk_bs, dv_bs, softmax_scale, q_prescaled, chain_ws, chain_ws_bytes
+extern "C" int BWD_ENTRY(BWD_ARGS_DECL) { return bwd_launch(BWD_ARGS, 0, stream); }
+extern "C" int VT_CAT(vt_attn_bwd_hd64_delta, VT_SUFFIX)(BWD_ARGS_DECL) { return bwd_launch(BWD_ARGS, 1, stream); }
+#undef BWD_ARGS
+#undef BWD_ARGS_DECL
+
 extern "C" long long VT_CAT(vt_attn_bwd_chain_ws_bytes, VT_SUFFIX)(int B, int H, int S) {
     if (B <= 0 || H <= 0 || S <= 0 || bwd_chain_len() <= 1) return 0;
     return bwd_chain_ws_bytes(g_bwd_slots);
diff --git a/videotuna-dev_amd/csrc/lora.hip b/videotuna-dev_amd/csrc/lora.hip
--- a/videotuna-dev_amd/csrc/lora.hip
+++ b/videotuna-dev_amd/csrc/lora.hip
@@ -304,6 +304,78 @@
                               void* stream) {
     return lora_up_add_launch(dX, ldx, dT, ldt, A, lda, R, M, K, nullptr, stream);
 }
+#define LU_ROWS 4
+template <typename F>
+__device__ __forceinline__ void lora_up_rows(float (&acc)[8], const bf16_t* dtrow, const bf16_t* acol, int lda, int r0, int r1,
+                                             F after_first_loads) {
+    int ri = r0;
+    for (; ri + LU_ROWS <= r1; ri += LU_ROWS) {
+        float t[LU_ROWS];
+        u32x4 ar[LU_ROWS];
+#pragma unroll
+        for (int u = 0; u < LU_ROWS; ++u) {
+            t[u] = bf2f(dtrow[ri + u]);
+            ar[u] = *(const u32x4*)(acol + (size_t)(ri + u) * lda);
+        }
+        if (ri == r0) after_first_loads();
+#pragma unroll
+        for (int u = 0; u < LU_ROWS; ++u) {
+            float a[8];
+            unpack8(ar[u], a);
+#pragma unroll
+            for (int q = 0; q < 8; ++q) acc[q] += t[u] * a[q];
+        }
+    }
+    for (; ri < r1; ++ri) {
+        const float t = bf2f(dtrow[ri]);
+        const u32x4 ar = *(const u32x4*)(acol + (size_t)ri * lda);
+        if (ri == r0) after_first_loads();
+        float a[8];
+        unpack8(ar, a);
+#pragma unroll
+        for (int q = 0; q < 8; ++q) acc[q] += t * a[q];
+    }
+}
+__global__ __launch_bounds__(256) void lora_up_add_delta_kernel(bf16_t* dX, int ldx, const bf16_t* dT, int ldt, const bf16_t* A, int lda,
+                                                               int R, long long M, int K, const bf16_t* O, int ldo, float* delta, int S) {
+    const int nch = K >> 3, H = K >> 6;
+    const long long total = M * nch;
+    for (long long i = (long long)blockIdx.x * 256 + threadIdx.x; i < total; i += (long long)gridDim.x * 256) {
+        const long long m = i / nch;
+        const int c = (int)(i - m * nch);
+        float v[8];
+        const u32x4 raw = *(const u32x4*)(dX + (size_t)m * ldx + c * 8);
+        const u32x4 oraw = *(const u32x4*)(O + (size_t)m * ldo + c * 8);
+        lora_up_rows(v, dT + (size_t)m * ldt, A + c * 8, lda, 0, R, [&] { unpack8(raw, v); });
+        const u32x4 packed = pack8(v);
+        *(u32x4*)(dX + (size_t)m * ldx + c * 8) = packed;
+        float fa[8], fc[8];
+        unpack8(oraw, fa);
+        unpack8(packed, fc);
+        float acc = 0.f;
+#pragma unroll
+        for (int q = 0; q < 8; ++q) acc += fa[q] * fc[q];
+        acc += __shfl_xor(acc, 1, 64);
+        acc += __shfl_xor(acc, 2, 64);
+        acc += __shfl_xor(acc, 4, 64);
+        if ((c & 7) == 0) {
+            const long long b = m / S;
+            const int s = (int)(m - b * S);
+            delta[((size_t)b * H + (c >> 3)) * S + s] = acc;
+        }
+    }
+}
+extern "C" int vt_lora_up_add_delta(void* dX, int ldx, const void* dT, int ldt, const void* A, int lda, int R, long long M, int K,
+                                    const void* O, int ldo, float* delta, int S, void* stream) {
+    if (M <= 0 || K <= 0 || (K % 64) || R <= 0 || R > 16 || (ldx % 8) || (lda % 8) || ldx < K || ldt < R) return VT_ERR_BAD_SHAPE;
+    if (O == nullptr || delta == nullptr || (ldo % 8) || ldo < K || S <= 0 || (M % S)) return VT_ERR_BAD_SHAPE;
+    if ((((uintptr_t)dX) | ((uintptr_t)A) | ((uintptr_t)O)) & 15) return VT_ERR_BAD_ALIGN;
+    long long total = M * (K >> 3), b = (total + 255) / 256;
+    const dim3 grid((unsigned)(b > 8192 ? 8192 : b));
+    hipLaunchKernelGGL(lora_up_add_delta_kernel, grid, dim3(256), 0, (hipStream_t)stream, (bf16_t*)dX, ldx, (const bf16_t*)dT, ldt,
+                       (const bf16_t*)A, lda, R, M, K, (const bf16_t*)O, ldo, delta, S);
+    return hipGetLastError() == hipSuccess ? VT_OK : VT_ERR_LAUNCH;
+}
 extern "C" int vt_lora_up_add_drop(void* dX, int ldx, const void* dT, int ldt, const void* A, int lda, int R, int n_adapters, long long M,
                                    int K, float p, unsigned long long seed, int site0, void* stream) {
     if (lora_drop_args_bad(R, n_adapters, p, site0)) return VT_ERR_BAD_SHAPE;
diff --git a/videotuna-dev_amd/csrc/norm.hip b/videotuna-dev_amd/csrc/norm.hip
--- a/videotuna-dev_amd/csrc/norm.hip
+++ b/videotuna-dev_amd/csrc/norm.hip
@@ -121,9 +121,11 @@
     const bf16_t* dres; int lddres;
     bf16_t* dx; int lddx;
     int M, D, S, St;
+    const float* gate_txt; const float* gate_vid; int gate_bstride;
+    bf16_t* gated; int ldg;
 };
 
-template <int NCH>
+template <int NCH, bool GATE = false>
 __global__ __launch_bounds__(256) void ln_modulate_bwd_kernel(LnBwdParams p) {
     const int lane = threadIdx.x & 63;
     const int m = blockIdx.x * 4 + (threadIdx.x >> 6);
@@ -136,6 +138,12 @@
         const int s = m - b * p.S;
         scp = (s < p.St ? p.scale_txt : p.scale_vid) + (size_t)b * p.mod_bstride;
     }
+    const float* gp = nullptr;
+    if constexpr (GATE) {
+        const int b = m / p.S;
+        const int s = m - b * p.S;
+        gp = (s < p.St ? p.gate_txt : p.gate_vid) + (size_t)b * p.gate_bstride;
+    }
     float gv[NCH][8], xh[NCH][8];
     float s1 = 0.f, s2 = 0.f;
 #pragma unroll
@@ -184,7 +192,16 @@
 #pragma unroll
                 for (int j = 0; j < 8; ++j) o[j] += dr[j];
             }
-            *(u32x4*)(p.dx + (size_t)m * p.lddx + c * 8) = pack8(o);
+            const u32x4 packed = pack8(o);
+            *(u32x4*)(p.dx + (size_t)m * p.lddx + c * 8) = packed;
+            if constexpr (GATE) {
+                float v[8];
+                unpack8(packed, v);
+                f32x4 a = *(const f32x4*)(gp + c * 8), bq = *(const f32x4*)(gp + c * 8 + 4);
+#pragma unroll
+                for (int j = 0; j < 4; ++j) { v[j] *= a[j]; v[j + 4] *= bq[j]; }
+                *(u32x4*)(p.gated + (size_t)m * p.ldg + c * 8) = pack8(v);
+            }
         }
     }
 }
@@ -234,24 +251,51 @@
     return hipGetLastError() == hipSuccess ? VT_OK : VT_ERR_LAUNCH;
 }
 
-extern "C" int vt_ln_modulate_bwd(const void* dy, int lddy, const void* x, int ldx, const float* mean, const float* rstd,
+static int ln_modulate_bwd_launch(const void* dy, int lddy, const void* x, int ldx, const float* mean, const float* rstd,
                                   const void* gamma, const float* scale_txt, const float* scale_vid, int mod_bstride,
-                                  const void* dres, int lddres, void* dx, int lddx,
-                                  int M, int D, int S, int St, void* stream) {
+                                  const void* dres, int lddres, void* dx, int lddx, int M, int D, int S, int St,
+                                  const float* gate_txt, const float* gate_vid, int gate_bstride, void* gated, int ldg, void* stream) {
     if (M <= 0 || D <= 0 || (D % 8) || D > 4096 || (ldx % 8) || (lddy % 8) || (lddx % 8)) return VT_ERR_BAD_SHAPE;
     if (dres != nullptr && (lddres % 8)) return VT_ERR_BAD_SHAPE;
     if (scale_vid != nullptr && (scale_txt == nullptr || (mod_bstride % 4))) return VT_ERR_BAD_SHAPE;
     if ((((uintptr_t)x) | ((uintptr_t)dy) | ((uintptr_t)dx) | ((uintptr_t)dres)) & 15) return VT_ERR_BAD_ALIGN;
     LnBwdParams p{(const bf16_t*)dy, lddy, (const bf16_t*)x, ldx, mean, rstd, (const bf16_t*)gamma,
                   scale_txt, scale_vid, mod_bstride, (const bf16_t*)dres, lddres, (bf16_t*)dx, lddx,
-                  M, D, S > 0 ? S : 1, St};
+                  M, D, S > 0 ? S : 1, St, gate_txt, gate_vid, gate_bstride, (bf16_t*)gated, ldg};
     dim3 grid((M + 3) / 4), block(256);
     hipStream_t st = (hipStream_t)stream;
     const int nch = nch_for(D);
-    if (nch <= 1) hipLaunchKernelGGL(ln_modulate_bwd_kernel<1>, grid, block, 0, st, p);
-    else if (nch <= 4) hipLaunchKernelGGL(ln_modulate_bwd_kernel<4>, grid, block, 0, st, p);
-    else hipLaunchKernelGGL(ln_modulate_bwd_kernel<8>, grid, block, 0, st, p);
+    if (gate_txt == nullptr) {
+        if (nch <= 1) hipLaunchKernelGGL(ln_modulate_bwd_kernel<1>, grid, block, 0, st, p);
+        else if (nch <= 4) hipLaunchKernelGGL(ln_modulate_bwd_kernel<4>, grid, block, 0, st, p);
+        else hipLaunchKernelGGL(ln_modulate_bwd_kernel<8>, grid, block, 0, st, p);
+    } else {
+        if (nch <= 1) hipLaunchKernelGGL((ln_modulate_bwd_kernel<1, true>), grid, block, 0, st, p);
+        else if (nch <= 4) hipLaunchKernelGGL((ln_modulate_bwd_kernel<4, true>), grid, block, 0, st, p);
+        else hipLaunchKernelGGL((ln_modulate_bwd_kernel<8, true>), grid, block, 0, st, p);
+    }
     return hipGetLastError() == hipSuccess ? VT_OK : VT_ERR_LAUNCH;
+}
+
+extern "C" int vt_ln_modulate_bwd(const void* dy, int lddy, const void* x, int ldx, const float* mean, const float* rstd,
+                                  const void* gamma, const float* scale_txt, const float* scale_vid, int mod_bstride,
+                                  const void* dres, int lddres, void* dx, int lddx,
+                                  int M, int D, int S, int St, void* stream) {
+    return ln_modulate_bwd_launch(dy, lddy, x, ldx, mean, rstd, gamma, scale_txt, scale_vid, mod_bstride, dres, lddres, dx, lddx,
+                                  M, D, S, St, nullptr, nullptr, 0, nullptr, 0, stream);
+}
+
+extern "C" int vt_ln_modulate_bwd_gate(const void* dy, int lddy, const void* x, int ldx, const float* mean, const float* rstd,
+                                       const void* gamma, const float* scale_txt, const float* scale_vid, int mod_bstride,
+                                       const void* dres, int lddres, void* dx, int lddx, int M, int D, int S, int St,
+                                       const float* gate_txt, const float* gate_vid, int gate_bstride, void* gated_out, int ldg,
+                                       void* stream) {
+    if (gate_txt == nullptr || gate_vid == nullptr || gated_out == nullptr || (gate_bstride % 4) || (ldg % 8) || ldg < D || S <= 0 ||
+        St < 0 || St > S)
+        return VT_ERR_BAD_SHAPE;
+    if ((((uintptr_t)gate_txt) | ((uintptr_t)gate_vid) | ((uintptr_t)gated_out)) & 15) return VT_ERR_BAD_ALIGN;
+    return ln_modulate_bwd_launch(dy, lddy, x, ldx, mean, rstd, gamma, scale_txt, scale_vid, mod_bstride, dres, lddres, dx, lddx,
+                                  M, D, S, St, gate_txt, gate_vid, gate_bstride, gated_out, ldg, stream);
 }
 
 __global__ __launch_bounds__(256) void qk_layernorm_fwd_kernel(const bf16_t* qkv, int ld, bf16_t* out, int ldo,
diff --git a/videotuna-dev_amd/engine.py b/videotuna-dev_amd/engine.py
--- a/videotuna-dev_amd/engine.py
+++ b/videotuna-dev_amd/engine.py
@@ -271,9 +271,10 @@
             ops.skinny_tn_drop(x, dt, nj * r, nj, g, 1, d, 1.0, d, *drop, site + j)
 
 
-def _lora_dx(st, i, proj, dxe, d, drop=None):
+def _lora_dx(st, i, proj, dxe, d, drop=None, delta=None):
     n, a, _, site = _lora_proj(st, i, proj, st.flat_bf16)
     r = st.r
+    assert delta is None or (not st.wide and drop is None and n * r <= 16)
     if st.wide:
         if drop is None:
             ops.lora_up_add_wide(dxe, dxe[:, d:], a, n, r, st.rp, d)
@@ -282,9 +283,21 @@
         return
     for j, nj in _narrow_calls(n, r):
         if drop is None:
-            ops.lora_up_add(dxe, dxe[:, d + j * r:], a[j * r:(j + nj) * r], nj * r, d)
+            if delta is None:
+                ops.lora_up_add(dxe, dxe[:, d + j * r:], a[j * r:(j + nj) * r], nj * r, d)
+            else:
+                ops.lora_up_add_delta(dxe, dxe[:, d + j * r:], a[j * r:(j + nj) * r], nj * r, d, *delta)
         else:
             ops.lora_up_add_drop(dxe, dxe[:, d + j * r:], a[j * r:(j + nj) * r], nj * r, nj, d, *drop, site + j)
+
+
+def _lora_tail_fused() -> bool:
+    import os
+    return os.environ.get("VT355_LORA_TAIL", "1") != "0"
+
+
+def _lora_dx_delta_ok(st, drop) -> bool:
+    return not st.wide and drop is None and "to_out.0" in st.targets
 
 
 def _lora_dx_dgelu(st, i, du, dt, u, K, drop):
@@ -517,12 +530,16 @@
     delta = E(B * H * S, dt=torch.float32)
     chain_ws = ops.attn_bwd_chain_workspace(B, H, S, dev)
     dh_in = E(M, d)
+    fused = _lora_tail_fused()
+    pre_delta = fused and _lora_dx_delta_ok(st, drop)
+    gated = False
     for i in reversed(range(L)):
         Lw, a = P.layers[i], ctx.blocks[i]
         if ctx.recompute:
             _, a = block_forward(model, i, a.h_in, mod, ctx.dims, ctx.rope, True, ctx.scratch, drop)
         m1, m2 = _mod(mod, 2 * i, d), _mod(mod, 2 * i + 1, d)
-        ops.gate_mul(dh, tgf, m2.gate_txt, m2.gate_vid, m2.bs, d, S, St)
+        if not gated:
+            ops.gate_mul(dh, tgf, m2.gate_txt, m2.gate_vid, m2.bs, d, S, St)
         if ff2:
             ops.gemm(tgf, Lw.w2_bt, tgf[:, d:], None, K=d)
             _lora_db(st, tn, tgf, a.g[:, dff:], st.view(st.grad, i, "B", 5), d, Lw.c_2 if dora else None)
@@ -543,20 +560,22 @@
                 _dora_dm(st, i, 4, du, a.u, Lw.b1)
             _lora_da(st, i, "ff1", a.x2, dx2, d, drop)
             _lora_dx(st, i, "ff1", dx2, d, drop)
-        ops.ln_modulate_bwd(dx2, a.h1, a.mean2, a.rstd2, Lw.n2g, (m2.scale_txt, m2.scale_vid, m2.bs), dh, dh1, d, S, St)
-        ops.gate_mul(dh1, tg, m1.gate_txt, m1.gate_vid, m1.bs, d, S, St)
+        ops.ln_modulate_bwd(dx2, a.h1, a.mean2, a.rstd2, Lw.n2g, (m2.scale_txt, m2.scale_vid, m2.bs), dh, dh1, d, S, St,
+                            gate=(m1.gate_txt, m1.gate_vid, m1.bs, tg) if fused else None)
+        if not fused:
+            ops.gate_mul(dh1, tg, m1.gate_txt, m1.gate_vid, m1.bs, d, S, St)
         ops.gemm(tg, Lw.w_o_t, dO, None)
         out_adapted = dora and "to_out.0" in st.targets
         _lora_db(st, tn, tg, a.o[:, d:], st.b_out(st.grad, i), d, Lw.c_o if out_adapted else None)
         if out_adapted:
             _dora_dm(st, i, 3, tg, a.ao, Lw.b_o)
         _lora_da(st, i, "out", a.o, dO, d, drop)
-        _lora_dx(st, i, "out", dO, d, drop)
+        _lora_dx(st, i, "out", dO, d, drop, delta=(a.o, delta, S) if pre_delta else None)
         dq.zero_()
         qk3, qkv3 = a.qkh.view(B, S, 2 * d), a.qkv.view(B, S, 3 * d)
         ops.attn_bwd(qk3[:, :, :d], qk3[:, :, d:], qkv3[:, :, 2 * d:], a.o.view(B, S, d + eo)[:, :, :d],
                      dO.view(B, S, d + eo)[:, :, :d], a.lse, delta, dq, dkh.view(B, S, d),
-                     dqkv.view(B, S, 3 * d)[:, :, 2 * d:], B, H, S, q_prescaled=True, chain_ws=chain_ws)
+                     dqkv.view(B, S, 3 * d)[:, :, 2 * d:], B, H, S, q_prescaled=True, chain_ws=chain_ws, have_delta=pre_delta)
         ops.qk_layernorm_bwd(dq.view(M, d), dkh, a.qkv, a.qmean, a.qrstd, Lw.gq, Lw.gk, dqkv, H, rope=ctx.rope)
         if i > 0:
             ops.gemm(dqkv, Lw.w_qkv_t, dx1, None)
@@ -569,8 +588,10 @@
         _lora_da(st, i, "qkv", a.x1, dx1, d, drop)
         if i > 0:
             _lora_dx(st, i, "qkv", dx1, d, drop)
+            mp = _mod(mod, 2 * i - 1, d)
             ops.ln_modulate_bwd(dx1, a.h_in, a.mean1, a.rstd1, Lw.n1g, (m1.scale_txt, m1.scale_vid, m1.bs), dh1, dh_in,
-                                d, S, St)
+                                d, S, St, gate=(mp.gate_txt, mp.gate_vid, mp.bs, tgf) if fused else None)
+            gated = fused
             dh, dh_in = dh_in, dh
         ctx.blocks[i] = None
     return None
diff --git a/videotuna-dev_amd/ops.py b/videotuna-dev_amd/ops.py
--- a/videotuna-dev_amd/ops.py
+++ b/videotuna-dev_amd/ops.py
@@ -402,7 +402,7 @@
 
 
 def attn_bwd(q, k, v, o, do, lse2, delta_ws, dq_f32, dk, dv, B: int, H: int, S: int, scale: Optional[float] = None,
-             q_prescaled: bool = False, chain_ws: Optional[torch.Tensor] = None, _entry=None):
+             q_prescaled: bool = False, chain_ws: Optional[torch.Tensor] = None, _entry=None, have_delta: bool = False):
     scale = 1.0 / math.sqrt(64) if scale is None else scale
     for n, t in (("q", q), ("k", k), ("v", v), ("o", o), ("do", do), ("dk", dk), ("dv", dv)):
         _req(t, BF16, n, 3)
@@ -410,7 +410,7 @@
     lib = load_library()
 
     def launch(ws, fn=None):
-        check((fn or lib.vt_attn_bwd_hd64)(q.data_ptr(), k.data_ptr(), v.data_ptr(), o.data_ptr(), do.data_ptr(),
+        check((fn or (lib.vt_attn_bwd_hd64_delta if have_delta else lib.vt_attn_bwd_hd64))(q.data_ptr(), k.data_ptr(), v.data_ptr(), o.data_ptr(), do.data_ptr(),
                                lse2.data_ptr(), delta_ws.data_ptr(), dq_f32.data_ptr(), dk.data_ptr(), dv.data_ptr(),
                                B, H, S,
                                q.stride(1), k.stride(1), v.stride(1), o.stride(1), do.stride(1),
@@ -445,10 +445,21 @@
                                      x.shape[0], D, S, St, eps, _stream()), "vt_ln_modulate_fwd")
 
 
-def ln_modulate_bwd(dy, x, mean, rstd, gamma, scales, dres, dx, D: int, S: int, St: int):
+def ln_modulate_bwd(dy, x, mean, rstd, gamma, scales, dres, dx, D: int, S: int, St: int, gate=None):
     _req(dy, BF16, "dy", 2); _req(x, BF16, "x", 2); _req(dx, BF16, "dx", 2)
     sc = (None, None, 0) if scales is None else scales
     lib = load_library()
+    if gate is not None:
+        g_txt, g_vid, g_bs, gated = gate
+        _req(gated, BF16, "gated_out", 2)
+        if gated.shape[0] != x.shape[0] or gated.shape[1] < D:
+            raise ValueError(f"ln_modulate_bwd: gated_out {tuple(gated.shape)} for {x.shape[0]} rows of {D}")
+        with _timed_hbm("ln_modulate_bwd", x.shape[0], (8.0 if dres is None else 10.0) * x.shape[0] * D):
+            check(lib.vt_ln_modulate_bwd_gate(dy.data_ptr(), dy.stride(0), x.data_ptr(), x.stride(0), mean.data_ptr(), rstd.data_ptr(),
+                                              _p(gamma), _p(sc[0]), _p(sc[1]), sc[2], _p(dres), 0 if dres is None else dres.stride(0),
+                                              dx.data_ptr(), dx.stride(0), x.shape[0], D, S, St, g_txt.data_ptr(), g_vid.data_ptr(), g_bs,
+                                              gated.data_ptr(), gated.stride(0), _stream()), "vt_ln_modulate_bwd_gate")
+        return
     with _timed_hbm("ln_modulate_bwd", x.shape[0], (6.0 if dres is None else 8.0) * x.shape[0] * D):
         check(lib.vt_ln_modulate_bwd(dy.data_ptr(), dy.stride(0), x.data_ptr(), x.stride(0), mean.data_ptr(), rstd.data_ptr(),
                                      _p(gamma), _p(sc[0]), _p(sc[1]), sc[2], _p(dres), 0 if dres is None else dres.stride(0),
@@ -603,6 +614,15 @@
     _req(dx, BF16, "dx", 2); _req(dt, BF16, "dt", 2); _req(a, BF16, "a", 2)
     check(load_library().vt_lora_up_add(dx.data_ptr(), dx.stride(0), dt.data_ptr(), dt.stride(0), a.data_ptr(), a.stride(0),
                                         R, dx.shape[0], K, _stream()), "vt_lora_up_add")
+
+
+def lora_up_add_delta(dx, dt, a, R: int, K: int, o, delta, S: int):
+    _req(dx, BF16, "dx", 2); _req(dt, BF16, "dt", 2); _req(a, BF16, "a", 2); _req(o, BF16, "o", 2); _req(delta, torch.float32, "delta")
+    if o.shape[0] != dx.shape[0] or o.shape[1] < K or delta.numel() < dx.shape[0] * (K // 64) or not delta.is_contiguous():
+        raise ValueError(f"lora_up_add_delta: o {tuple(o.shape)}, delta {tuple(delta.shape)} for dx {tuple(dx.shape)}, K {K}")
+    check(load_library().vt_lora_up_add_delta(dx.data_ptr(), dx.stride(0), dt.data_ptr(), dt.stride(0), a.data_ptr(), a.stride(0),
+                                              R, dx.shape[0], K, o.data_ptr(), o.stride(0), delta.data_ptr(), S, _stream()),
+          "vt_lora_up_add_delta")
 
 
 def lora_pack_b(bcat_f32, wext, ldw: int, n_adapters: int, d_out: int, r: int, scale: float):
```
